# Farama-Foundation/Miniworld

Measured on AMD Instinct MI355X. Metric: env-steps/s (batched, 80x60 RGB), higher is better.
Workload: dtype f32

## Files before the change

include/mwengine.h:

```cpp
#ifndef MWENGINE_H
#define MWENGINE_H
#include <stdint.h>
#ifdef __cplusplus
extern "C" {
#endif

#define MW_ABI_VERSION 4

enum {
    MW_OK = 0,
    MW_E_INVALID = -1,
    MW_E_HIP = -2,
    MW_E_NOMEM = -3,
    MW_E_CAPACITY = -4,
    MW_E_DEVICE = -5,
    MW_E_OVERFLOW = -6
};

enum { MW_ENT_NONE = 0, MW_ENT_BOX = 1, MW_ENT_MESH = 2, MW_ENT_FRAME = 3 };

enum {
    MW_TASK_NONE = 0,
    MW_TASK_GOTO = 1,
    MW_TASK_PICKUP = 2,
// ... 126 lines not shown
typedef struct {
    int32_t n_rooms, n_tex, n_ops, n_ents;
    mw_prog_room rooms[MW_PROG_MAX_ROOMS];
    int32_t tex_nvar[MW_PROG_MAX_TEX];
    int32_t tex_var_id[MW_PROG_MAX_TEX][9];
    double tex_var_scale[MW_PROG_MAX_TEX][9][2];
    mw_prog_op ops[MW_PROG_MAX_OPS];
    int32_t ent_kind[MW_PROG_MAX_ENTS], ent_mesh[MW_PROG_MAX_ENTS], ent_static[MW_PROG_MAX_ENTS];
    double ent_pos[MW_PROG_MAX_ENTS][3], ent_dir[MW_PROG_MAX_ENTS], ent_geom[MW_PROG_MAX_ENTS][9];
    double colors[6][3];
    double extent[4];
    double street[4];
    int32_t sign_n, pad;
    int32_t sign_slot[8];
    double sign_reward[8];
} mw_gen_program;

int mw_set_gen_program(mw_engine *e, const mw_gen_program *prog, const mw_poly *polys, const int32_t *poly_room,
                       const int32_t *poly_surf, const double *poly_m , int32_t n_polys,
                       const double *segs, int32_t n_segs);

int mw_create(const mw_config *cfg, mw_engine **out);
void mw_destroy(mw_engine *e);
const char *mw_last_error(const mw_engine *e);

int mw_upload_texture(mw_engine *e, int32_t tex_id, const uint8_t *rgb_bottom_up, int32_t w, int32_t h);
int mw_upload_mesh(mw_engine *e, int32_t mesh_id, const float *pos, const float *nrm, const float *uv,
                   const float *rgb, int32_t ntris, int32_t tex_id);

int mw_set_geometry(mw_engine *e, int32_t env, const mw_poly *polys, int32_t n_polys,
                    const double *segs, int32_t n_segs);
int mw_get_geometry(mw_engine *e, int32_t env, mw_poly *polys, int32_t *n_polys, double *segs, int32_t *n_segs);
int mw_set_state(mw_engine *e, int32_t first_env, int32_t count, const mw_state_view *host);
int mw_set_step_params(mw_engine *e, const double *host_params);
int mw_get_state(mw_engine *e, int32_t first_env, int32_t count, mw_state_view *host);
int mw_reset(mw_engine *e, const uint8_t *mask, const uint64_t *seeds, void *stream);

int mw_step(mw_engine *e, const int32_t *d_actions, uint8_t *d_obs, float *d_depth,
            float *d_reward, uint8_t *d_term, uint8_t *d_trunc, void *stream);
#define MW_MAX_REPEAT 256
int mw_step_repeat(mw_engine *e, const int32_t *d_actions, int32_t repeat, uint8_t *d_obs, float *d_depth,
                   float *d_reward, uint8_t *d_term, uint8_t *d_trunc, int32_t *d_nsteps, void *stream);
int mw_set_final_obs(mw_engine *e, uint8_t *d_final_obs, float *d_final_depth);
#define MW_MAX_STACK 16
enum { MW_STACK_PAD_RESET = 0, MW_STACK_PAD_ZERO = 1 };
int mw_set_frame_stack(mw_engine *e, int32_t depth, int32_t pad, uint8_t *d_ring, uint8_t *d_final_stack );
int mw_stack_refresh(mw_engine *e, const uint8_t *d_obs, void *stream);
int mw_stack_window(const mw_engine *e, int32_t *first_slot, int64_t *pushes);
enum { MW_OBS_HWC_U8 = 0, MW_OBS_CWH_U8 = 1, MW_OBS_GREY_F64 = 2 };
int mw_set_obs_layout(mw_engine *e, int32_t layout);

int mw_pcg64_draws(uint64_t seed, int32_t n, const int32_t *bounds, double *out);

int mw_selftest_rcp(unsigned long long *bad_per_exp, uint32_t *examples, uint32_t *n);
int mw_selftest_div(unsigned long long *n_bad, uint32_t *examples);
int mw_selftest_sort(const uint32_t *keys, const int32_t *n, int32_t blocks, uint16_t *order);
int mw_selftest_q(unsigned long long *n_bad, uint32_t *examples);
int mw_selftest_sincosf(unsigned long long *sums, unsigned long long n64, unsigned long long *sums64);

int mw_render(mw_engine *e, uint8_t *d_obs, float *d_depth, void *stream);
int mw_render_top(mw_engine *e, uint8_t *d_obs, float *d_depth, int32_t render_agent, void *stream);
int mw_render_view(mw_engine *e, int32_t env, int32_t view_flags, int32_t width, int32_t height, int32_t msaa,
                   uint8_t *d_out, float *d_depth, void *stream);
int mw_visible_ents(mw_engine *e, int32_t first_env, int32_t count, uint8_t *d_vis, void *stream);

int64_t mw_snapshot_bytes(const mw_engine *e, int32_t capacity);
int mw_snapshot_save(mw_engine *e, const int32_t *d_envs, int32_t count, uint8_t *d_snap, int32_t capacity, void *stream);
int mw_snapshot_load(mw_engine *e, const int32_t *d_envs, const int32_t *d_recs, int32_t count,
                     const uint8_t *d_snap, int32_t n_recs, int32_t capacity, void *stream);

int mw_check(mw_engine *e, void *stream);

int mw_kernel_time_ms(mw_engine *e, int32_t reset, double *raster_ms, double *setup_ms, int64_t *launches);

int mw_get_info(mw_engine *e, int32_t *d_health, double *d_ent_pos, int32_t ent_slot, void *stream);
int mw_get_final_info(mw_engine *e, int32_t *d_health, double *d_goal_pos, void *stream);
int mw_get_reset_pending(mw_engine *e, uint8_t *d_out, void *stream);

int mw_set_frame_reuse(mw_engine *e, int32_t on);
int mw_get_frame_clean(mw_engine *e, uint8_t *d_out, void *stream);

int mw_set_frame_cache(mw_engine *e, int32_t slots);
int mw_get_frame_source(mw_engine *e, uint8_t *d_out, void *stream);

int mw_get_list_lengths(mw_engine *e, int32_t first_env, int32_t count, int32_t *host_out, void *stream);

int mw_debug_set_mesh_frame_seq(mw_engine *e, uint32_t seq);
int mw_debug_get_slow_heads(mw_engine *e, uint32_t *host_out, void *stream);

enum { MW_PATH_TILE = 0, MW_PATH_QUAD = 1, MW_PATH_QUAD_MESH = 2, MW_PATH_GENERIC = 3 };
int mw_raster_path(const mw_engine *e);

#ifdef __cplusplus
}
#endif
#endif
```

miniworld_amd/csrc/mw_engine.hip:

```cpp
#include <hip/hip_runtime.h>

#include <algorithm>
#include <cmath>
#include <cstdarg>
#include <cstdio>
#include <cstdlib>
#include <cstring>
#include <memory>
#include <string>
#include <utility>
#include <vector>

#include "mw_assets.h"
#include "mw_device.h"
#include "mw_kernels.h"
#include "mw_rng.h"

#define MW_TIMING_STRIDE 8

extern "C" __global__ void mw_info_kernel(int N, int E, const int32_t *health, const double *epos, int slot, int32_t *out_health, double *out_pos)
{
    const int i = blockIdx.x * blockDim.x + threadIdx.x;
    if (i >= N) return;
    if (out_health) out_health[i] = health[i];
// ... 54 lines not shown
struct Destroy { void operator()(H h) const { (void)destroy(h); } };
template <typename T>
using DevBuf = std::unique_ptr<T, Destroy<void *, hipFree>>;
using Stream = std::unique_ptr<ihipStream_t, Destroy<hipStream_t, hipStreamDestroy>>;
using Event = std::unique_ptr<ihipEvent_t, Destroy<hipEvent_t, hipEventDestroy>>;
}

struct mw_engine {
    mw_config cfg{};
    MwArgs args{};
    MwArgs *d_gen_live = nullptr, *d_gen_spare = nullptr;
    bool spare_mode = false;
    bool side_refill_pending = false;
    MwSpare spare_host{};
    int32_t *d_spare_dummy = nullptr;
    int n_sets = 1;
    std::string err;
    std::vector<DevBuf<void>> fixed;
    std::vector<MwTexDesc> tex_desc;
    std::vector<std::vector<uint32_t>> tex_data;
    DevBuf<uint32_t> d_texels;
    size_t texel_cap = 0;
    MwMeshDesc *d_meshdesc = nullptr;
    std::vector<mwasset::HostMesh> meshes;
    struct MeshPools {
        DevBuf<float> pos, nrm, rgb, uv;
        DevBuf<float> stream, attr;
        DevBuf<float4> vpos;
        DevBuf<uint2> idx;
    } pools;
    int max_mesh_verts = 0, max_mesh_tris = 0;
    bool have_meshes = false, visible_attr_set = false;
    Stream side_stream;
    Event ev_fork;
    struct MeshPath {
        Stream quad_stream;
        Event ev_fork, ev_join;
        DevBuf<uint32_t> view_keys;
        size_t view_keys_bytes = 0;
        DevBuf<uint32_t> keys;
        bool keys_dirty = true;
        DevBuf<int32_t> slow_count;
        int32_t *ent_counter = nullptr;
        DevBuf<uint32_t> slow_envs;
        DevBuf<uint32_t> tile_list;
        DevBuf<uint32_t> ent_list;
        int ent_list_cap = 0;
        uint32_t frame_seq = 1;
        DevBuf<uint32_t> slow_tris; DevBuf<float4> slow_frags; DevBuf<uint32_t> slow_head;
        DevBuf<float> plane_cache;
        int plane_cap = 0;
        static constexpr int mesh_tile_waves = 16384;
        static constexpr int ent_blocks = 512;
        static constexpr int slow_waves = 8192;
    } mp;
    int obs_layout = MW_OBS_HWC_U8;
    float *d_reward_scratch = nullptr;
    uint8_t *d_flag_scratch = nullptr;
    int32_t *d_action_scratch = nullptr;
    uint8_t *d_mask = nullptr;
    double *d_step_override = nullptr;
    bool use_step_override = false;
    bool timing = false;
    int timing_stride = MW_TIMING_STRIDE;
    uint64_t frame_count = 0;
    struct Ev { Event a, b, c; };
    std::vector<Ev> ev_used, ev_free;
    int waves_per_env = 0;
    DevBuf<MwProgram> d_prog;
    DevBuf<mw_poly> d_prog_polys;
    DevBuf<int32_t> d_prog_room, d_prog_surf;
    DevBuf<double> d_prog_m, d_prog_segs;
    int texel_bytes = 4;
    int dbg_flags = 0;
    int last_raster_path = -1;
    bool use_k2q = true;
    bool k2q_ok = false;
    bool generic_raster = false;
    unsigned long long *d_ent_prof = nullptr;
    unsigned long long *d_k2q_prof = nullptr;
    uint8_t *final_obs = nullptr;
    float *final_depth = nullptr;
    int32_t *d_final_list = nullptr;
    bool frame_reuse = false;
    struct { uint8_t *obs = nullptr; float *depth = nullptr; int layout = 0; bool valid = false; } held;
    struct {
        int slots = 0;
        DevBuf<uint8_t> frames;
        DevBuf<float> depth;
        DevBuf<uint64_t> meta;
        DevBuf<MwFcArgs> d_args;
        MwFcArgs args{};
        bool args_stale = true;
        bool with_depth = false;
        bool dirty = true;
    } fc;
    struct {
        int depth = 0, pad = 0, layout = 0, cur = 0;
        uint8_t *ring = nullptr, *final_stack = nullptr;
        size_t frame_bytes = 0;
        int64_t pushes = 0;
        uint8_t *flags = nullptr;
    } stack;
    MwSnapConfig snap_cfg{};
    MwSnapLayout snap_layout{};
    MwSnapTable *d_snap_tab = nullptr;
    int snap_chunks_per_item = 0;
    Event ev_refill_done;
};

namespace {

int fail(mw_engine *e, int code, const char *fmt, ...)
{
    char buf[512];
    va_list ap;
    va_start(ap, fmt);
    vsnprintf(buf, sizeof buf, fmt, ap);
    va_end(ap);
    if (e) e->err = buf; else g_create_error = buf;
    return code;
}

#define HIP_TRY(e, call)                                                                         \
    do {                                                                                         \
        hipError_t _st = (call);                                                                 \
        if (_st != hipSuccess)                                                                   \
            return fail(e, MW_E_HIP, "%s failed: %s (%s:%d)", #call, hipGetErrorString(_st), __FILE__, __LINE__); \
    } while (0)

template <typename T>
int dev_alloc(mw_engine *e, DevBuf<T> &out, size_t count, bool zero = true)
{
    void *p = nullptr;
    const size_t bytes = std::max<size_t>(count, 1) * sizeof(T);
    hipError_t st = hipMalloc(&p, bytes);
    if (st != hipSuccess) return fail(e, MW_E_NOMEM, "hipMalloc(%zu) failed: %s", bytes, hipGetErrorString(st));
    DevBuf<T> buf(static_cast<T *>(p));
    if (zero) {
        st = hipMemset(p, 0, bytes);
        if (st != hipSuccess) return fail(e, MW_E_HIP, "hipMemset failed: %s", hipGetErrorString(st));
    }
    out = std::move(buf);
    return MW_OK;
}

template <typename T>
int fixed_alloc(mw_engine *e, T **out, size_t count)
{
    DevBuf<T> buf;
    if (const int rc = dev_alloc(e, buf, count)) return rc;
    *out = buf.get();
    e->fixed.emplace_back(std::move(buf));
    return MW_OK;
}

template <typename T, typename C>
int grow(mw_engine *e, DevBuf<T> &buf, C &have, C want, size_t unit)
{
    if (want <= have) return MW_OK;
    DevBuf<T> fresh;
    if (const int rc = dev_alloc(e, fresh, (size_t)want * unit / sizeof(T), false)) return rc;
    (void)hipDeviceSynchronize();
    buf = std::move(fresh);
    have = want;
    return MW_OK;
}

hipError_t make_event(Event &out, unsigned flags = hipEventDisableTiming)
{
    hipEvent_t ev = nullptr;
    const hipError_t st = hipEventCreateWithFlags(&ev, flags);
    if (st == hipSuccess) out.reset(ev);
    return st;
}

hipError_t make_stream(Stream &out)
{
    int prio_least = 0, prio_greatest = 0;
    (void)hipDeviceGetStreamPriorityRange(&prio_least, &prio_greatest);
    hipStream_t s = nullptr;
    const hipError_t st = hipStreamCreateWithPriority(&s, hipStreamNonBlocking, prio_least);
    if (st == hipSuccess) out.reset(s);
    return st;
}

auto k1_of(const mw_engine *e, int lanes) -> decltype(&mw_step_setup_kernel)
{
    const bool pcg = e->cfg.rng_mode == MW_RNG_PCG64;
    if (lanes) return pcg ? mw_step_setup_dense_pcg_kernel : mw_step_setup_dense_kernel;
    return pcg ? mw_step_setup_pcg_kernel : mw_step_setup_kernel;
}

auto k1_repeat_of(const mw_engine *e, int lanes) -> decltype(&mw_step_repeat_kernel)
{
    const bool pcg = e->cfg.rng_mode == MW_RNG_PCG64;
    if (lanes) return pcg ? mw_step_repeat_dense_pcg_kernel : mw_step_repeat_dense_kernel;
    return pcg ? mw_step_repeat_pcg_kernel : mw_step_repeat_kernel;
}

template <typename... A>
struct KernelPair {
    void (*plain)(A...);
    void (*sub)(A..., const int32_t *);
};
template <typename... A>
KernelPair<A...> kernel_pair(void (*plain)(A...), void (*sub)(A..., const int32_t *)) { return {plain, sub}; }
#define MW_PAIR(stem) kernel_pair(stem##_kernel, stem##_sub_kernel)

template <typename... A, typename... P>
void launch(const KernelPair<A...> &k, const int32_t *list, dim3 grid, dim3 block, size_t lds, hipStream_t st, P &&...args)
{
    if (list) hipLaunchKernelGGL(k.sub, grid, block, lds, st, std::forward<P>(args)..., list);
    else hipLaunchKernelGGL(k.plain, grid, block, lds, st, std::forward<P>(args)...);
}

auto geom_kernel_of(int L, int msaa)
{
    const bool fixed8 = msaa == 8;
    if (L == 64) return fixed8 ? MW_PAIR(mw_geom_big) : MW_PAIR(mw_geom_big_any);
    return fixed8 ? MW_PAIR(mw_geom) : MW_PAIR(mw_geom_any);
}

auto tile_kernel_of(bool big, bool depth, bool general, bool ragged, bool mesh, bool first)
{
    if (mesh) {
        if (big) return MW_PAIR(mw_raster_big_mesh_wrap);
        if (general) return MW_PAIR(mw_raster_mesh_wrap);
        if (first) return depth ? MW_PAIR(mw_raster_nomesh_depth) : MW_PAIR(mw_raster_nomesh);
        return depth ? MW_PAIR(mw_raster_mesh_depth) : MW_PAIR(mw_raster_mesh);
    }
    if (ragged) return big ? MW_PAIR(mw_raster_big_ragged) : MW_PAIR(mw_raster_ragged);
    if (general) return big ? MW_PAIR(mw_raster_big_wrap) : MW_PAIR(mw_raster_wrap);
    if (big) return depth ? MW_PAIR(mw_raster_big_depth) : MW_PAIR(mw_raster_big);
    return depth ? MW_PAIR(mw_raster_depth) : MW_PAIR(mw_raster);
}

#define MW_DEBUG_BITS 0xFCCF
int raster_flags(const mw_engine *e, int part, uint32_t stamp, bool reuse = false)
{
    return e->dbg_flags | e->obs_layout << 8 | part << 4 | (int)(stamp << 16) | (reuse && stamp == 0u ? MW_RASTER_REUSE : 0);
}
void drop_held_frame(mw_engine *e) { e->held.valid = false; }
void drop_frame_cache(mw_engine *e) { e->fc.dirty = true; }

size_t obs_row_bytes(const mw_engine *e)
{
    return (size_t)e->cfg.obs_width * e->cfg.obs_height * (e->obs_layout == MW_OBS_GREY_F64 ? 8 : 3);
}

int stack_phase(const mw_engine *e) { return (int)((e->stack.pushes + e->stack.depth - 1) % e->stack.depth); }
uint8_t *stack_flags(const mw_engine *e, int half) { return e->stack.flags + (size_t)half * e->cfg.num_envs; }
int stack_check(mw_engine *e, const char *what)
{
    if (e->stack.depth && (e->stack.layout != e->obs_layout || e->stack.frame_bytes != obs_row_bytes(e)))
        return fail(e, MW_E_INVALID, "%s: the frame stack was set under obs layout %d, the engine is in layout %d now (mw_set_frame_stack again, or switch back)",
                    what, e->stack.layout, e->obs_layout);
    return MW_OK;
}
int launch_stack(mw_engine *e, bool push, const uint8_t *d_obs, const uint8_t *term, const uint8_t *trunc, hipStream_t st)
{
    auto &s = e->stack;
    const int N = e->cfg.num_envs, phase = push ? (int)(s.pushes % s.depth) : stack_phase(e);
    const bool installs = e->cfg.generator != MW_GEN_NONE;
    const bool same = installs && e->cfg.autoreset == MW_AUTORESET_SAME_STEP, next = installs && e->cfg.autoreset == MW_AUTORESET_NEXT_STEP;
    const uint8_t *final_obs = push && same && s.final_stack ? e->final_obs : nullptr;
    uint8_t *final_stack = final_obs ? s.final_stack : nullptr;
    const bool wide = (((uintptr_t)d_obs | (uintptr_t)s.ring | (uintptr_t)final_obs | (uintptr_t)final_stack | (uintptr_t)s.frame_bytes) & 15u) == 0;
    const size_t units = s.frame_bytes / (wide ? 16 : 1), chunk = (size_t)MW_STACK_THREADS * MW_STACK_UNROLL;
    const dim3 grid(N, (unsigned)((units + chunk - 1) / chunk));
    const uint8_t *in = stack_flags(e, s.cur);
    uint8_t *out = stack_flags(e, s.cur ^ 1);
    if (push)
        hipLaunchKernelGGL(mw_stack_push_kernel, grid, dim3(MW_STACK_THREADS), 0, st, s.depth, s.pad, phase, (unsigned long long)s.frame_bytes, (int)wide, d_obs, s.ring,
                           in, out, same ? term : nullptr, same ? trunc : nullptr, next ? (const uint8_t *)e->args.reset_pending : nullptr, final_obs, final_stack);
    else
        hipLaunchKernelGGL(mw_stack_refresh_kernel, grid, dim3(MW_STACK_THREADS), 0, st, s.depth, s.pad, phase, (unsigned long long)s.frame_bytes, (int)wide, d_obs, s.ring,
                           in, out);
    HIP_TRY(e, hipGetLastError());
    s.cur ^= 1;
    if (push) ++s.pushes;
    return MW_OK;
}

bool tile_kernels_exact(int W, int H) { return W <= 128 && H <= 128 && W * H <= 128 * 96; }

bool frame_on_grid(int W, int H) { return W % MW_TILE_W == 0 && H % MW_TILE_H == 0; }
bool tile_path_ok(int W, int H) { return frame_on_grid(W, H) && tile_kernels_exact(W, H); }
bool frame_size_ok(int W, int H)
{
    return W >= 1 && H >= 1 && W <= 255 * MW_TILE_W && H <= 255 * MW_TILE_H;
}

int geom_lanes(const mw_engine *e)
{
    const int items = 2 * (e->cfg.max_polys + 6 * e->cfg.max_ents + 1);
    int L = 8;
    while (L < items && L < 64) L <<= 1;
    if (L == 32) L = 16;
    if (L == 64 && !e->args.rec_order && e->cfg.max_polys <= 64) L = 32;
#if defined(MW_PERF_HOOKS) || defined(MW_TUNE_HOOKS)
    if (const char *s = getenv("MW_GEOM_LANES")) { const int v = atoi(s); if ((v == 8 || v == 16 || v == 32 || v == 64) && v >= L) L = v; }
#endif
    return L;
}

// ... 135 lines not shown
}

struct RasterPath {
    int path;
    bool mesh;
    bool quad4;
    bool big, general, ragged, depth;
};
RasterPath raster_path(const mw_engine *e, bool depth)
{
    const MwArgs &a = e->args; const int S = e->cfg.msaa;
    RasterPath p{MW_PATH_GENERIC, false, false, a.rec_order != nullptr, e->obs_layout != MW_OBS_HWC_U8 || e->dbg_flags != 0, !frame_on_grid(a.W, a.H), depth};
    const bool k2q = e->use_k2q && e->k2q_ok && !p.big && !(S == 4 && (e->have_meshes || e->generic_raster));
    const bool ragged_tiles = !e->have_meshes && p.ragged && a.H % 2 == 0 && tile_kernels_exact(a.tiles_x * MW_TILE_W, a.tiles_y * MW_TILE_H);
    p.quad4 = k2q && S == 4;
    const bool generic = S != 8 || (!tile_path_ok(a.W, a.H) && !ragged_tiles);
    p.mesh = !p.quad4 && !generic && e->have_meshes;
    p.path = p.quad4 ? MW_PATH_QUAD : generic ? MW_PATH_GENERIC : !k2q ? MW_PATH_TILE : p.mesh ? MW_PATH_QUAD_MESH : MW_PATH_QUAD;
    return p;
}

int ensure_mesh_buffers(mw_engine *e)
{
    const MwArgs &a = e->args; mw_engine::MeshPath &m = e->mp;
    const size_t N = (size_t)e->cfg.num_envs;
    if (!m.quad_stream) HIP_TRY(e, make_stream(m.quad_stream));
    for (Event *ev : {&m.ev_fork, &m.ev_join}) if (!*ev) HIP_TRY(e, make_event(*ev));
    if (raster_path(e, false).path == MW_PATH_GENERIC)
        return grow(e, m.view_keys, m.view_keys_bytes, N * a.W * a.H * e->cfg.msaa * 4, 1);
    if (a.W > 255 * MW_TILE_W || a.H > 255 * MW_TILE_H) return fail(e, MW_E_CAPACITY, "frame too large for the mesh tile rectangles");
    if (a.n_tiles > 255 || a.n_tiles > 32 * geom_lanes(e))
        return fail(e, MW_E_CAPACITY, "%d tiles per frame: the mesh tiles' work list holds 255 (8-bit tile index) and 32 per lane of the geometry kernel (%d lanes)", a.n_tiles, geom_lanes(e));
    const long long want = std::min<long long>(0xC000, (long long)e->cfg.max_ents * e->max_mesh_tris);
    int rc;
    if ((rc = grow(e, m.plane_cache, m.plane_cap, (int)want, N * (MW_PLANE_REC + MW_PLANE_XTRA) * 4))) return rc;
    if (!m.ent_list) {
        const int cap = (int)N * std::min(MW_MAX_MESH_ENTS, std::max(e->cfg.max_ents, 1));
        DevBuf<uint32_t> ents, slow, tiles;
        if ((rc = dev_alloc(e, ents, (size_t)cap * 16, false)) || (rc = dev_alloc(e, slow, N * 2, false)) ||
            (rc = dev_alloc(e, tiles, N * (size_t)a.n_tiles * 8, false)))
            return rc;
        m.ent_list_cap = cap;
        m.ent_list = std::move(ents); m.slow_envs = std::move(slow); m.tile_list = std::move(tiles);
    }
    if (!m.keys) {
        const size_t px = N * a.W * a.H;
        DevBuf<uint32_t> keys, tris, head; DevBuf<int32_t> cnt; DevBuf<float4> frags;
        if ((rc = dev_alloc(e, keys, px * 8, false)) || (rc = dev_alloc(e, cnt, N * 4 + 2 * MW_CNT_WORDS)) ||
            (rc = dev_alloc(e, tris, N * MW_SLOW_TRIS, false)) || (rc = dev_alloc(e, frags, N * MW_SLOW_STRIDE, false)) ||
            (rc = dev_alloc(e, head, px)))
            return rc;
        HIP_TRY(e, hipMemset(keys.get(), 0xFF, px * 8 * 4));
        m.ent_counter = cnt.get() + N * 4;
        m.keys = std::move(keys); m.slow_count = std::move(cnt); m.slow_tris = std::move(tris);
        m.slow_frags = std::move(frags); m.slow_head = std::move(head);
        (void)hipDeviceSynchronize();
        m.keys_dirty = false;
    }
    return MW_OK;
}

struct MeshFrame {
    uint32_t stamp;
    int parity;
    int32_t *cnt, *cnt_next, *slow_count;
    uint32_t *slow_envs;
};
MeshFrame mesh_frame(mw_engine::MeshPath &m, size_t N)
{
    const uint32_t seq = m.frame_seq++;
    const int parity = (int)(seq & 1u);
    return {seq & 0xFFFFu, parity, m.ent_counter + parity * MW_CNT_WORDS, m.ent_counter + (parity ^ 1) * MW_CNT_WORDS,
            m.slow_count.get() + (size_t)parity * 2 * N, m.slow_envs.get() + (size_t)parity * N};
}

enum { FRAME_ALL = 0, FRAME_TERMINAL = 1, FRAME_LIST = 2 };

struct Frame {
    MwArgs a;
    int view_flags;
    const int32_t *list;
    uint8_t *obs; float *depth; hipStream_t st; bool reuse;
    int fc_slots;
    uint8_t *source;
    RasterPath p;
    MeshFrame mf;
};

void launch_step_and_geometry(mw_engine *e, const Frame &f, bool do_step, int frame, bool async_refill, const int32_t *d_actions,
                              float *d_reward, uint8_t *d_term, uint8_t *d_trunc, int repeat, int32_t *d_nsteps)
{
    const MwArgs &a = f.a; const int N = e->cfg.num_envs;
    if (do_step) {
        const int refill_blocks = (e->spare_mode && !async_refill) ? (N + 63) / 64 : 0;
        MwArgs ak = a;
        if (frame == FRAME_TERMINAL) ak.autoreset = MW_AUTORESET_NEXT_STEP;
        const int lanes = k1_dense_lanes(e), epw = lanes ? 64 / lanes : 1;
        const dim3 grid((N + epw - 1) / epw + refill_blocks);
        float *reward = d_reward ? d_reward : e->d_reward_scratch;
        uint8_t *term = d_term ? d_term : e->d_flag_scratch, *trunc = d_trunc ? d_trunc : e->d_flag_scratch + N;
        if (repeat > 0) hipLaunchKernelGGL(k1_repeat_of(e, lanes), grid, dim3(64), 0, f.st, ak, lanes, d_actions, reward, term, trunc, repeat, d_nsteps);
        else hipLaunchKernelGGL(k1_of(e, lanes), grid, dim3(64), 0, f.st, ak, lanes, d_actions, reward, term, trunc);
    }
    if (frame == FRAME_TERMINAL)
        hipLaunchKernelGGL(mw_final_list_kernel, dim3(1), dim3(1024), 0, f.st, N, (const uint8_t *)a.reset_pending, a.pending_remove, e->d_final_list);
    const int L = geom_lanes(e), epw = 64 / L;
    launch(geom_kernel_of(L, e->cfg.msaa), f.list, dim3((N + epw - 1) / epw), dim3(64), 0, f.st, a, f.view_flags, e->cfg.msaa, L, N);
    if (do_step && e->cfg.task == MW_TASK_COLLECT)
        hipLaunchKernelGGL(e->cfg.rng_mode == MW_RNG_PCG64 ? mw_collect_respawn_pcg_kernel : mw_collect_respawn_kernel, dim3((N + 63) / 64), dim3(64), 0, f.st, a);
}

int launch_side_refill(mw_engine *e, hipStream_t st)
{
    if (!e->side_stream) HIP_TRY(e, make_stream(e->side_stream));
    if (!e->ev_fork) HIP_TRY(e, make_event(e->ev_fork));
    HIP_TRY(e, hipEventRecord(e->ev_fork.get(), st));
    HIP_TRY(e, hipStreamWaitEvent(e->side_stream.get(), e->ev_fork.get(), 0));
    hipLaunchKernelGGL(e->cfg.rng_mode == MW_RNG_PCG64 ? mw_refill_pcg_kernel : mw_refill_kernel, dim3(e->cfg.num_envs), dim3(64), 0, e->side_stream.get(), e->args);
    e->side_refill_pending = true;
    return MW_OK;
}

int launch_generic(mw_engine *e, const MwArgs &a, int first_env, int count, int S, dim3 mesh_grid, uint8_t *out, float *depth,
                   int layout, const int32_t *list, hipStream_t st)
{
    uint32_t *keys = nullptr;
    if (e->have_meshes) {
        const size_t need = (size_t)count * a.W * a.H * S * 4;
        if (need > e->mp.view_keys_bytes) return fail(e, MW_E_INVALID, "view keys missing (mw_upload_mesh allocates them)");
        keys = e->mp.view_keys.get();
        HIP_TRY(e, hipMemsetAsync(keys, 0xFF, need, st));
        launch(MW_PAIR(mw_view_mesh), list, mesh_grid, dim3(256), 0, st, a.W, a.H, S, first_env, (const float *)a.envhdr, a.mesh_pos, keys);
    }
    const bool any = !frame_on_grid(a.W, a.H) || layout != MW_OBS_HWC_U8;
    launch(any ? MW_PAIR(mw_view_raster_any) : MW_PAIR(mw_view_raster), list, dim3(a.n_tiles, count), dim3(64), 0, st, first_env, a.W, a.H, S,
           a.max_vis, a.tiles_x, (const float *)a.rec_raster, (const float *)a.rec_shade, (const float *)a.rec_cull, (const int32_t *)a.nvis,
           (const float *)a.envhdr, a.tex, a.texels, a.mesh_pos, a.mesh_nrm, a.mesh_rgb, a.mesh_uv, keys, out, depth, e->texel_bytes, layout);
    return MW_OK;
}

void launch_quad(const mw_engine *e, const Frame &f, int part, hipStream_t st)
{
    const MwArgs &a = f.a;
    const int lds = mw_rasterq_lds_bytes(e->cfg.msaa, a.W, a.H, a.n_tiles, f.depth ? 1 : 0);
    launch(f.p.quad4 ? MW_PAIR(mw_rasterq4) : MW_PAIR(mw_rasterq), f.list, dim3(e->cfg.num_envs), dim3(MWQ_THREADS), (size_t)lds, st, a.N, a.W, a.H, a.max_vis,
           a.tiles_x, a.n_tiles, (const float *)a.rec_raster, (const float *)a.rec_shade, (const float *)a.rec_cull,
           (const int32_t *)a.nvis, (const float *)a.envhdr, a.texels, f.obs, f.depth, raster_flags(e, part, 0u, f.reuse), e->texel_bytes, e->d_k2q_prof,
           (const uint8_t *)a.frame_clean, f.fc_slots ? (const MwFcArgs *)e->fc.d_args.get() : nullptr, f.source);
}

void launch_tiles(const mw_engine *e, const Frame &f, int part, hipStream_t st)
{
    const MwArgs &a = f.a; const mw_engine::MeshPath &m = e->mp;
    const int N = e->cfg.num_envs, wpe = e->waves_per_env;
    const int lds_recs = a.max_vis < MW_LDS_RECS ? a.max_vis : MW_LDS_RECS;
    const size_t lds = f.p.big ? 192 : (size_t)lds_recs * (MW_LDS_SHADE_Q + MW_LDS_CULL_Q) * 16 + 192;
    const bool listed = part == 2 && a.tile_list != nullptr;
    if (listed) part = 3;
    const int wpe2 = part == 2 ? a.n_tiles : wpe;
    const int tpw2 = part == 2 ? 1 : (a.n_tiles + wpe - 1) / wpe;
    const int grid = listed ? std::min(m.mesh_tile_waves, N * (int)a.n_tiles) : (N + 7) / 8 * 8 * wpe2;
    launch(tile_kernel_of(f.p.big, f.p.depth, f.p.general, f.p.ragged, f.p.mesh, part == 1), f.list, dim3(grid), dim3(64), lds, st,
           a.N, a.W, a.H, a.max_vis, a.tiles_x, a.n_tiles, wpe2, tpw2, (const float *)a.rec_raster, (const float *)a.rec_shade,
           (const float *)a.rec_cull, (const int32_t *)a.nvis, (const float *)a.envhdr, a.tex, a.texels, f.obs, f.depth, raster_flags(e, part, f.mf.stamp, f.reuse),
           e->texel_bytes, (const uint16_t *)a.rec_order, a.mesh_pos, a.mesh_nrm, a.mesh_rgb, a.mesh_uv, m.keys.get(),
           (const float *)m.plane_cache.get(), m.plane_cap, (const float4 *)m.slow_frags.get(), (const uint32_t *)m.slow_head.get(),
           (const uint32_t *)a.tile_list, a.ent_list_n, a.tile_list_cap, std::max(a.n_xcc, 1), (const uint8_t *)a.frame_clean);
}

int launch_mesh_chain(mw_engine *e, const Frame &f, hipStream_t st)
{
    const MwArgs &a = f.a; const MeshFrame &mf = f.mf;
    mw_engine::MeshPath &m = e->mp; const int N = e->cfg.num_envs;
    if (!m.keys || !m.plane_cache || !m.quad_stream) return fail(e, MW_E_INVALID, "mesh buffers missing (mw_upload_mesh allocates them)");
    if (m.keys_dirty) HIP_TRY(e, hipMemsetAsync(m.keys.get(), 0xFF, (size_t)N * a.W * a.H * 8 * 4, st));
    m.keys_dirty = true;
    if (mf.stamp == 0u) HIP_TRY(e, hipMemsetAsync(m.slow_head.get(), 0, (size_t)N * a.W * a.H * 4, st));
    HIP_TRY(e, hipEventRecord(m.ev_fork.get(), st));
    HIP_TRY(e, hipStreamWaitEvent(m.quad_stream.get(), m.ev_fork.get(), 0));
    hipLaunchKernelGGL(mw_mesh_entity_kernel, dim3(std::max(a.n_xcc, std::min(m.ent_list_cap, m.ent_blocks))), dim3(MW_ENT_THREADS), (size_t)e->max_mesh_verts * 16, st, N, a.W, a.H,
                       (const float *)a.envhdr, a.mesh, (const float4 *)e->pools.vpos.get(), (const uint2 *)e->pools.idx.get(), (const float *)e->pools.stream.get(),
                       (const float *)e->pools.attr.get(), m.keys.get(), m.plane_cache.get(), m.plane_cap, mf.slow_count, m.slow_tris.get(),
                       (const uint32_t *)m.ent_list.get(), m.ent_list_cap, mf.cnt, mf.cnt_next, mf.slow_envs, e->args.n_xcc, e->d_ent_prof);
    hipLaunchKernelGGL(mw_mesh_slow_kernel, dim3(std::min(N * 16, m.slow_waves)), dim3(64), 0, st, a.W, a.H, (const float *)a.envhdr, a.mesh_pos, a.mesh_nrm, a.mesh_rgb,
                       a.mesh_uv, a.texels, e->texel_bytes, m.keys.get(), m.slow_count.get(), N, mf.parity, (const uint32_t *)m.slow_tris.get(),
                       m.slow_frags.get(), m.slow_head.get(), mf.stamp, a.status,
                       (const uint32_t *)mf.slow_envs, (const int32_t *)(mf.cnt + MW_CNT_SLOW_ENVS));
    if (f.p.path == MW_PATH_QUAD_MESH) launch_quad(e, f, 1, m.quad_stream.get()); else launch_tiles(e, f, 1, m.quad_stream.get());
    launch_tiles(e, f, 2, st);
    HIP_TRY(e, hipEventRecord(m.ev_join.get(), m.quad_stream.get()));
    HIP_TRY(e, hipStreamWaitEvent(st, m.ev_join.get(), 0));
    m.keys_dirty = false;
    return MW_OK;
}

int launch_frame(mw_engine *e, bool do_step, int view_flags, const int32_t *d_actions, uint8_t *d_obs, float *d_depth,
                 float *d_reward, uint8_t *d_term, uint8_t *d_trunc, hipStream_t st, int frame = FRAME_ALL, int repeat = 0,
                 int32_t *d_nsteps = nullptr)
{
    if (!d_obs) return fail(e, MW_E_INVALID, "d_obs is null");
    const bool plain = frame == FRAME_ALL && view_flags == 0;
    const bool reuse = e->frame_reuse && plain && do_step && !e->have_meshes && e->dbg_flags == 0 && e->held.valid && e->held.obs == d_obs &&
                       e->held.depth == d_depth && e->held.layout == e->obs_layout;
    drop_held_frame(e);
    const int N = e->cfg.num_envs;
    Frame f{e->args, view_flags, frame == FRAME_LIST ? e->d_final_list : nullptr, d_obs, d_depth, st, reuse, 0, nullptr, raster_path(e, d_depth != nullptr), {}};
    if (plain && do_step && f.p.path == MW_PATH_QUAD) {
        f.source = f.a.fc_source;
        if (e->fc.slots > 0 && e->fc.frames && !e->have_meshes && e->dbg_flags == 0 && e->obs_layout == MW_OBS_HWC_U8 && e->cfg.task != MW_TASK_COLLECT) {
            if (d_depth && !e->fc.depth) {
                if (const int rc = dev_alloc(e, e->fc.depth, (size_t)N * e->fc.slots * f.a.W * f.a.H, false)) return rc;
                e->fc.args_stale = true;
            }
            if ((d_depth != nullptr) != e->fc.with_depth) { e->fc.with_depth = d_depth != nullptr; drop_frame_cache(e); }
            if (e->fc.args_stale) {
                e->fc.args = MwFcArgs{f.a.fc_key, e->fc.meta.get(), e->fc.frames.get(), e->fc.depth.get(), e->fc.slots, 0};
                HIP_TRY(e, hipMemcpyAsync(e->fc.d_args.get(), &e->fc.args, sizeof(MwFcArgs), hipMemcpyHostToDevice, st));
                e->fc.args_stale = false;
                drop_frame_cache(e);
            }
            if (e->fc.dirty) {
                HIP_TRY(e, hipMemsetAsync(e->fc.meta.get(), 0, (size_t)N * MW_FC_META_WORDS(e->fc.slots) * 8, st));
                e->fc.dirty = false;
            }
            f.fc_slots = e->fc.slots;
        }
    }
    f.a.step_override = e->use_step_override ? e->d_step_override : nullptr;
    if (f.p.mesh && e->mp.ent_list && e->mp.keys) {
        f.mf = mesh_frame(e->mp, (size_t)N);
        f.a.ent_list = e->mp.ent_list.get(); f.a.ent_list_n = f.mf.cnt; f.a.ent_list_cap = e->mp.ent_list_cap;
        f.a.tile_list = e->mp.tile_list.get(); f.a.tile_list_cap = N * f.a.n_tiles;
    }
    mw_engine::Ev ev{};
    const bool timed = frame != FRAME_LIST && e->timing && (e->frame_count++ % (uint64_t)e->timing_stride) == 0;
    if (timed) {
        ev = get_events(e);
        (void)hipEventRecord(ev.a.get(), st);
    }
    const bool async_refill = e->spare_mode && do_step && e->cfg.generator == MW_GEN_MAZE;
    launch_step_and_geometry(e, f, do_step, frame, async_refill, d_actions, d_reward, d_term, d_trunc, repeat, d_nsteps);
    if (timed) (void)hipEventRecord(ev.b.get(), st);
    int rc = MW_OK;
    if (async_refill && (rc = launch_side_refill(e, st))) return rc;
    if (f.p.path == MW_PATH_GENERIC) rc = launch_generic(e, f.a, 0, N, e->cfg.msaa, dim3(32, N), d_obs, d_depth, e->obs_layout, f.list, st);
    else if (f.p.mesh) rc = launch_mesh_chain(e, f, st);
    else if (f.p.path == MW_PATH_QUAD) launch_quad(e, f, 0, st);
    else launch_tiles(e, f, 0, st);
    if (rc) return rc;
    e->last_raster_path = f.p.path;
    if (timed) {
        (void)hipEventRecord(ev.c.get(), st);
        e->ev_used.push_back(std::move(ev));
    }
    HIP_TRY(e, hipGetLastError());
    if (plain) e->held = {d_obs, d_depth, e->obs_layout, true};
    return MW_OK;
}

int init_engine(mw_engine *e, const mw_config *cfg)
{
    e->cfg = *cfg;
    const int N = cfg->num_envs, E = std::max(cfg->max_ents, 1);
    e->cfg.max_ents = E;
    e->n_sets = cfg->shared_geometry ? 1 : N;
    MwArgs &a = e->args;
    a.N = N; a.W = cfg->obs_width; a.H = cfg->obs_height; a.E = E;
    a.max_polys = cfg->max_polys; a.max_segs = cfg->max_segs;
    a.max_vis = cfg->max_visible * 6 < 60000 ? cfg->max_visible * 6 : 60000;
    a.shared_geom = cfg->shared_geometry ? 1 : 0;
    a.task = cfg->task; a.goal_ent = cfg->goal_ent; a.goal_ent2 = cfg->goal_ent2; a.num_objs = cfg->num_objs; a.max_steps = cfg->max_episode_steps;
    a.rng_mode = cfg->rng_mode;
    a.occlusion = 1;
    if (const char *s = getenv("MW_OCCLUSION")) a.occlusion = atoi(s) != 0;
    a.domain_rand = cfg->domain_rand; a.generator = cfg->generator; a.autoreset = cfg->autoreset;
    a.tiles_x = (a.W + MW_TILE_W - 1) / MW_TILE_W; a.tiles_y = (a.H + MW_TILE_H - 1) / MW_TILE_H; a.n_tiles = a.tiles_x * a.tiles_y;
    a.agent_radius = cfg->agent_radius; a.max_forward_step = cfg->max_forward_step;
    a.agent_height = cfg->agent_height > 0.0 ? cfg->agent_height : 1.6;
    a.fwd = cfg->forward_step; a.drift = cfg->forward_drift; a.turn = cfg->turn_step;
    memcpy(a.gen_args, cfg->gen_args, sizeof a.gen_args);
    MwGenTables gt{};
    memcpy(gt.gen_tab, cfg->gen_tab, sizeof gt.gen_tab);
    memcpy(gt.gen_colors, cfg->gen_colors, sizeof gt.gen_colors);
    memcpy(gt.tex_nvar, cfg->tex_nvar, sizeof gt.tex_nvar);
    memcpy(gt.tex_var_id, cfg->tex_var_id, sizeof gt.tex_var_id);
    memcpy(gt.tex_var_scale, cfg->tex_var_scale, sizeof gt.tex_var_scale);
    gt.room_wall_height = cfg->room_wall_height; gt.room_no_ceiling = cfg->room_no_ceiling;
    for (int i = 0; i < 3; ++i) {
        a.sky[i] = cfg->sky_color[i]; a.light_pos[i] = cfg->light_pos[i]; a.light_color[i] = cfg->light_color[i];
        a.light_ambient[i] = cfg->light_ambient[i]; a.color_bias[i] = cfg->obj_color_bias[i];
    }
    a.cam_height = cfg->cam_height; a.cam_fwd_disp = cfg->cam_fwd_disp; a.cam_pitch = cfg->cam_pitch; a.cam_fov_y = cfg->cam_fov_y;
#define ALLOC(ptr, count) do { if (const int rc_ = fixed_alloc(e, &ptr, (size_t)(count))) return rc_; } while (0)
    ALLOC(a.ax, N); ALLOC(a.ay, N); ALLOC(a.az, N); ALLOC(a.adir, N);
    ALLOC(a.cam, 4 * (size_t)N); ALLOC(a.light, 12 * (size_t)N);
    ALLOC(a.carry, N); ALLOC(a.step, N); ALLOC(a.picked, N);
    if (cfg->task == MW_TASK_COLLECT) { ALLOC(a.health, N); ALLOC(a.final_health, N); }
    ALLOC(a.final_goal, 3 * (size_t)N);
    ALLOC(a.ekind, (size_t)E * N); ALLOC(a.emesh, (size_t)E * N); ALLOC(a.estatic, (size_t)E * N);
    ALLOC(a.epos, 3 * (size_t)E * N); ALLOC(a.edir, (size_t)E * N); ALLOC(a.egeom, 9 * (size_t)E * N);
    ALLOC(a.rng, 5 * (size_t)N); ALLOC(a.extent, 4 * (size_t)N);
    MwGenTables *d_gt = nullptr;
    ALLOC(d_gt, 1);
    HIP_TRY(e, hipMemcpy(d_gt, &gt, sizeof gt, hipMemcpyHostToDevice));
    a.gt = d_gt;
    mw_poly *polys = nullptr; int32_t *npolys = nullptr; double *segs = nullptr; int32_t *nsegs = nullptr;
    ALLOC(polys, (size_t)e->n_sets * cfg->max_polys); ALLOC(npolys, e->n_sets);
    ALLOC(segs, (size_t)e->n_sets * cfg->max_segs * 4); ALLOC(nsegs, e->n_sets);
    a.polys = polys; a.npolys = npolys; a.segs = segs; a.nsegs = nsegs;
    MwSpare sp{};
    {
        const bool small_scene = cfg->max_visible <= 64 && cfg->max_polys + 6 * std::max(cfg->max_ents, 1) <= 32;
        bool want = small_scene || cfg->generator == MW_GEN_MAZE;
        if (const char *s = getenv("MW_SPARE")) want = atoi(s) != 0;
        e->spare_mode = cfg->generator != MW_GEN_NONE && !cfg->domain_rand && want && cfg->task != MW_TASK_COLLECT;
    }
    if (e->spare_mode) {
        ALLOC(sp.ax, N); ALLOC(sp.ay, N); ALLOC(sp.az, N); ALLOC(sp.adir, N);
        ALLOC(sp.cam, 4 * (size_t)N); ALLOC(sp.light, 12 * (size_t)N); ALLOC(sp.extent, 4 * (size_t)N);
        ALLOC(sp.ekind, (size_t)E * N); ALLOC(sp.emesh, (size_t)E * N); ALLOC(sp.estatic, (size_t)E * N);
        ALLOC(sp.epos, 3 * (size_t)E * N); ALLOC(sp.edir, (size_t)E * N); ALLOC(sp.egeom, 9 * (size_t)E * N);
        if (!cfg->shared_geometry) {
            ALLOC(sp.polys, (size_t)e->n_sets * cfg->max_polys); ALLOC(sp.npolys, e->n_sets);
            ALLOC(sp.segs, (size_t)e->n_sets * cfg->max_segs * 4); ALLOC(sp.nsegs, e->n_sets);
        }
        MwSpare *d_sp = nullptr;
        ALLOC(d_sp, 1);
        ALLOC(a.refill_mask, N);
        ALLOC(e->d_spare_dummy, 3 * (size_t)N);
        e->spare_host = sp;
        {
            std::vector<uint32_t> ones((size_t)N, 1u);
            HIP_TRY(e, hipMemcpy(a.refill_mask, ones.data(), 4 * (size_t)N, hipMemcpyHostToDevice));
        }
        HIP_TRY(e, hipMemcpy(d_sp, &sp, sizeof sp, hipMemcpyHostToDevice));
        a.spare = d_sp;
    }
    if (cfg->generator != MW_GEN_NONE) {
        ALLOC(e->d_gen_live, 1); a.gen_live = e->d_gen_live;
        if (e->spare_mode) { ALLOC(e->d_gen_spare, 1); a.gen_spare = e->d_gen_spare; }
    }
    ALLOC(e->d_meshdesc, MW_MAX_MESH);
    a.mesh = e->d_meshdesc;
    ALLOC(a.rec_raster, (size_t)N * a.max_vis * MW_RASTER_REC);
    ALLOC(a.rec_shade, (size_t)N * a.max_vis * MW_SHADE_REC);
    ALLOC(a.rec_cull, (size_t)N * a.max_vis * MW_CULL_REC);
    if (cfg->max_visible > 64) {
        ALLOC(a.rec_order, (size_t)N * (a.max_vis + 1));
    }
    if (cfg->max_polys > 64 && !(getenv("MW_OCC_CACHE") && atoi(getenv("MW_OCC_CACHE")) == 0)) {
        ALLOC(a.occ_valid, e->n_sets);
        ALLOC(a.occ_cache, (size_t)e->n_sets * MW_OCC_CACHE_STRIDE(cfg->max_polys));
    }
    ALLOC(a.pending_remove, (size_t)N);
    ALLOC(a.reset_pending, (size_t)N);
    ALLOC(a.frame_clean, (size_t)N);
    ALLOC(a.fc_key, (size_t)MW_FC_KEY_WORDS * N); ALLOC(a.fc_epoch, (size_t)N); ALLOC(a.fc_source, (size_t)N);
    HIP_TRY(e, hipMemset(a.pending_remove, 0xFF, 4 * (size_t)N));
    ALLOC(a.nvis, N); ALLOC(a.envhdr, (size_t)MW_ENVHDR * N); ALLOC(a.status, 1);
    ALLOC(e->d_reward_scratch, N); ALLOC(e->d_flag_scratch, 2 * (size_t)N); ALLOC(e->d_action_scratch, N);
    ALLOC(e->d_final_list, 1 + (size_t)N);
    ALLOC(e->stack.flags, 2 * (size_t)N);
    ALLOC(e->d_mask, N); ALLOC(e->d_step_override, 3 * (size_t)N);
#ifdef MW_PERF_HOOKS
    if (getenv("MW_K1_PROF")) ALLOC(a.k1_prof, MW_K1_PROF_SLOTS * (size_t)N);
    if (getenv("MW_ENT_PROF")) ALLOC(e->d_ent_prof, (size_t)16 * 2 * N * MW_MAX_MESH_ENTS * 8);
    if (getenv("MW_K2Q_PROF")) ALLOC(e->d_k2q_prof, (size_t)N * 80);
#endif
#undef ALLOC
    {
        std::vector<int32_t> m1((size_t)N, -1);
        HIP_TRY(e, hipMemcpy(a.carry, m1.data(), 4 * (size_t)N, hipMemcpyHostToDevice));
        std::vector<uint64_t> seeds(5 * (size_t)N, 0);
        for (int i = 0; i < N; ++i) seed_env(e, seeds.data(), i, (uint64_t)i);
        HIP_TRY(e, hipMemcpy(a.rng, seeds.data(), 40 * (size_t)N, hipMemcpyHostToDevice));
    }
    e->meshes.assign(MW_MAX_MESH, {}); e->tex_desc.assign(MW_MAX_TEX, MwTexDesc{}); e->tex_data.assign(MW_MAX_TEX, {});
    if (const int rc = upload_textures(e)) return rc;
    e->waves_per_env = pick_waves_per_env(e);
    {
        uint32_t *p = nullptr, ids[256];
        a.n_xcc = 0;
        if (hipMalloc((void **)&p, sizeof ids) == hipSuccess) {
            const DevBuf<uint32_t> d_ids(p);
            hipLaunchKernelGGL(mw_xcc_probe_kernel, dim3(256), dim3(64), 0, 0, d_ids.get());
            if (hipMemcpy(ids, d_ids.get(), sizeof ids, hipMemcpyDeviceToHost) == hipSuccess) {
                uint32_t seen = 0u;
                for (uint32_t v : ids) seen |= 1u << (v & 15u);
                for (int n : {8, 4, 2}) if (seen == (1u << n) - 1u) a.n_xcc = n;
            }
        }
        if (a.n_xcc == 0) a.n_xcc = 1;
    }
    if (const char *s = getenv("MW_DEBUG_FLAGS")) e->dbg_flags = atoi(s) & MW_DEBUG_BITS;
    if (const char *s = getenv("MW_K2Q")) e->use_k2q = atoi(s) != 0;
    if (const char *s = getenv("MW_GENERIC_RASTER")) e->generic_raster = atoi(s) != 0;
    {
        const int S = cfg->msaa == 4 ? 4 : 8;
        const int lds = mw_rasterq_lds_bytes(S, a.W, a.H, a.n_tiles, 1);
        e->k2q_ok = (cfg->msaa == 8 || cfg->msaa == 4) && frame_on_grid(a.W, a.H) && a.W <= 128 && a.H <= 128 && a.W * a.H <= 8192 && lds <= 64 * 1024;
    }
    {
        e->snap_cfg = {E, cfg->max_polys, cfg->max_segs, cfg->shared_geometry ? 1 : 0, cfg->task, cfg->generator, cfg->rng_mode, e->spare_mode ? 1 : 0,
                       cfg->task == MW_TASK_COLLECT ? 1 : 0};
        const MwSnapLayout &L = e->snap_layout = mw_snap_layout(e->snap_cfg);
        void *arr[MW_SC_COUNT] = {};
        arr[MW_SC_AX] = a.ax; arr[MW_SC_AY] = a.ay; arr[MW_SC_AZ] = a.az; arr[MW_SC_ADIR] = a.adir; arr[MW_SC_CAM] = a.cam; arr[MW_SC_LIGHT] = a.light;
        arr[MW_SC_EXTENT] = a.extent; arr[MW_SC_CARRY] = a.carry; arr[MW_SC_STEP] = a.step; arr[MW_SC_PICKED] = a.picked; arr[MW_SC_HEALTH] = a.health;
        arr[MW_SC_FINAL_HEALTH] = a.final_health; arr[MW_SC_FINAL_GOAL] = a.final_goal; arr[MW_SC_EKIND] = a.ekind; arr[MW_SC_EMESH] = a.emesh;
        arr[MW_SC_ESTATIC] = a.estatic; arr[MW_SC_EPOS] = a.epos; arr[MW_SC_EDIR] = a.edir; arr[MW_SC_EGEOM] = a.egeom; arr[MW_SC_RNG] = a.rng;
        arr[MW_SC_PENDING_REMOVE] = a.pending_remove; arr[MW_SC_RESET_PENDING] = a.reset_pending;
        arr[MW_SC_NPOLYS] = const_cast<int32_t *>(a.npolys); arr[MW_SC_NSEGS] = const_cast<int32_t *>(a.nsegs);
        arr[MW_SC_SP_AX] = sp.ax; arr[MW_SC_SP_AY] = sp.ay; arr[MW_SC_SP_AZ] = sp.az; arr[MW_SC_SP_ADIR] = sp.adir; arr[MW_SC_SP_CAM] = sp.cam;
        arr[MW_SC_SP_LIGHT] = sp.light; arr[MW_SC_SP_EXTENT] = sp.extent; arr[MW_SC_SP_EKIND] = sp.ekind; arr[MW_SC_SP_EMESH] = sp.emesh;
        arr[MW_SC_SP_ESTATIC] = sp.estatic; arr[MW_SC_SP_EPOS] = sp.epos; arr[MW_SC_SP_EDIR] = sp.edir; arr[MW_SC_SP_EGEOM] = sp.egeom;
        arr[MW_SC_SP_NPOLYS] = sp.npolys; arr[MW_SC_SP_NSEGS] = sp.nsegs; arr[MW_SC_REFILL_MASK] = a.refill_mask;
        MwSnapTable t{};
        for (int id = 0; id < MW_SC_COUNT; ++id) {
            if (!L.comp_rows[id]) continue;
            if (!arr[id]) return fail(e, MW_E_INVALID, "snapshot layout: component %d has rows but no array", id);
            t.comp[t.n_comps++] = {arr[id], L.comp_unit[id], L.comp_row0[id], L.comp_rows[id], L.comp_elem[id], 0};
        }
        t.total_rows = L.total_rows; t.n_geo = L.n_geo; t.max_polys = cfg->max_polys; t.max_segs = cfg->max_segs;
        const int chunk = MW_SNAP_THREADS * MW_SNAP_UNROLL;
        t.poly_chunks = (cfg->max_polys * (MW_SNAP_POLY_BYTES / 16) + chunk - 1) / chunk;
        t.seg_chunks = (cfg->max_segs * (MW_SNAP_SEG_BYTES / 16) + chunk - 1) / chunk;
        t.eng_polys[0] = const_cast<mw_poly *>(a.polys); t.eng_segs[0] = const_cast<double *>(a.segs);
        t.eng_npolys[0] = const_cast<int32_t *>(a.npolys); t.eng_nsegs[0] = const_cast<int32_t *>(a.nsegs);
        t.eng_polys[1] = sp.polys; t.eng_segs[1] = sp.segs; t.eng_npolys[1] = sp.npolys; t.eng_nsegs[1] = sp.nsegs;
        t.polys_unit[0] = L.blob_unit[MW_SB_POLYS]; t.segs_unit[0] = L.blob_unit[MW_SB_SEGS];
        t.polys_unit[1] = L.blob_unit[MW_SB_SP_POLYS]; t.segs_unit[1] = L.blob_unit[MW_SB_SP_SEGS];
        t.npolys_unit[0] = L.comp_unit[MW_SC_NPOLYS]; t.nsegs_unit[0] = L.comp_unit[MW_SC_NSEGS];
        t.npolys_unit[1] = L.comp_unit[MW_SC_SP_NPOLYS]; t.nsegs_unit[1] = L.comp_unit[MW_SC_SP_NSEGS];
        t.reset_pending_unit = L.comp_unit[MW_SC_RESET_PENDING];
        e->snap_chunks_per_item = t.n_geo * (t.poly_chunks + t.seg_chunks);
        {
            std::vector<uint16_t> row_comp((size_t)t.total_rows);
            for (int c = 0; c < t.n_comps; ++c)
                for (int r = 0; r < t.comp[c].rows; ++r) row_comp[(size_t)t.comp[c].row0 + r] = (uint16_t)c;
            uint16_t *d_row_comp = nullptr;
            if (const int rc = fixed_alloc(e, &d_row_comp, row_comp.size())) return rc;
            HIP_TRY(e, hipMemcpy(d_row_comp, row_comp.data(), row_comp.size() * sizeof(uint16_t), hipMemcpyHostToDevice));
            t.row_comp = d_row_comp;
        }
// ... 601 lines not shown
    ON_DEVICE(e);
    HIP_TRY(e, hipStreamSynchronize((hipStream_t)stream));
    HIP_TRY(e, hipMemcpy(host_out, e->args.nvis + first_env, sizeof(int32_t) * (size_t)count, hipMemcpyDeviceToHost));
    return MW_OK;
}

int mw_get_info(mw_engine *e, int32_t *d_health, double *d_ent_pos, int32_t ent_slot, void *stream)
{
    if (!e) return MW_E_INVALID;
    if (!d_health && !d_ent_pos) return fail(e, MW_E_INVALID, "mw_get_info: nothing asked for");
    if (d_ent_pos && (ent_slot < 0 || ent_slot >= e->args.E)) return fail(e, MW_E_INVALID, "mw_get_info: entity slot %d out of range", ent_slot);
    if (d_health && !e->args.health) return fail(e, MW_E_INVALID, "mw_get_info: this engine's task keeps no health (MW_TASK_COLLECT only)");
    ON_DEVICE(e);
    const int N = e->cfg.num_envs;
    hipLaunchKernelGGL(mw_info_kernel, dim3((N + 255) / 256), dim3(256), 0, (hipStream_t)stream, N, e->args.E, (const int32_t *)e->args.health,
                       (const double *)e->args.epos, d_ent_pos ? ent_slot : 0, d_health, d_ent_pos);
    HIP_TRY(e, hipGetLastError());
    return MW_OK;
}

int mw_get_final_info(mw_engine *e, int32_t *d_health, double *d_goal_pos, void *stream)
{
    if (!e) return MW_E_INVALID;
    if (!d_health && !d_goal_pos) return fail(e, MW_E_INVALID, "mw_get_final_info: nothing asked for");
    if (d_health && !e->args.final_health) return fail(e, MW_E_INVALID, "mw_get_final_info: this engine's task keeps no health (MW_TASK_COLLECT only)");
    ON_DEVICE(e);
    const int N = e->cfg.num_envs;
    hipLaunchKernelGGL(mw_info_kernel, dim3((N + 255) / 256), dim3(256), 0, (hipStream_t)stream, N, 1, (const int32_t *)e->args.final_health,
                       (const double *)e->args.final_goal, 0, d_health, d_goal_pos);
    HIP_TRY(e, hipGetLastError());
    return MW_OK;
}

int mw_get_reset_pending(mw_engine *e, uint8_t *d_out, void *stream)
{
    if (!e) return MW_E_INVALID;
    if (!d_out) return fail(e, MW_E_INVALID, "mw_get_reset_pending: d_out is null");
    ON_DEVICE(e);
    HIP_TRY(e, hipMemcpyAsync(d_out, e->args.reset_pending, (size_t)e->cfg.num_envs, hipMemcpyDeviceToDevice, (hipStream_t)stream));
    return MW_OK;
}

int mw_set_frame_reuse(mw_engine *e, int32_t on)
{
    if (!e) return MW_E_INVALID;
    drop_held_frame(e);
    e->frame_reuse = on != 0;
    return MW_OK;
}

int mw_set_frame_cache(mw_engine *e, int32_t slots)
{
    if (!e) return MW_E_INVALID;
    if (slots < 0 || slots > MW_FC_MAX_SLOTS) return fail(e, MW_E_INVALID, "mw_set_frame_cache: %d slots outside 0 .. %d", (int)slots, MW_FC_MAX_SLOTS);
    ON_DEVICE(e);
    drop_frame_cache(e);
    if (slots == e->fc.slots) return MW_OK;
    HIP_TRY(e, hipDeviceSynchronize());
    e->fc.slots = 0;
    e->fc.frames.reset(); e->fc.depth.reset(); e->fc.meta.reset();
    if (slots > 0 && e->use_k2q && e->k2q_ok) {
        const size_t N = (size_t)e->cfg.num_envs;
        DevBuf<uint8_t> frames; DevBuf<uint64_t> meta;
        int rc;
        if ((rc = dev_alloc(e, frames, N * slots * e->cfg.obs_width * e->cfg.obs_height * 3, false)) || (rc = dev_alloc(e, meta, N * MW_FC_META_WORDS(slots))) ||
            (!e->fc.d_args && (rc = dev_alloc(e, e->fc.d_args, 1))))
            return rc;
        e->fc.frames = std::move(frames); e->fc.meta = std::move(meta);
        e->fc.args_stale = true;
    }
    e->fc.slots = slots;
    return MW_OK;
}

int mw_get_frame_source(mw_engine *e, uint8_t *d_out, void *stream)
{
    if (!e) return MW_E_INVALID;
    if (!d_out) return fail(e, MW_E_INVALID, "mw_get_frame_source: d_out is null");
    ON_DEVICE(e);
    HIP_TRY(e, hipMemcpyAsync(d_out, e->args.fc_source, (size_t)e->cfg.num_envs, hipMemcpyDeviceToDevice, (hipStream_t)stream));
    return MW_OK;
}

int mw_get_frame_clean(mw_engine *e, uint8_t *d_out, void *stream)
{
    if (!e) return MW_E_INVALID;
    if (!d_out) return fail(e, MW_E_INVALID, "mw_get_frame_clean: d_out is null");
    ON_DEVICE(e);
    HIP_TRY(e, hipMemcpyAsync(d_out, e->args.frame_clean, (size_t)e->cfg.num_envs, hipMemcpyDeviceToDevice, (hipStream_t)stream));
    return MW_OK;
}

int mw_kernel_time_ms(mw_engine *e, int32_t reset, double *raster_ms, double *setup_ms, int64_t *launches)
{
    if (!e) return MW_E_INVALID;
    ON_DEVICE(e);
    double r = 0, s = 0;
    int64_t n = 0;
    for (auto &ev : e->ev_used) {
        (void)hipEventSynchronize(ev.c.get());
        float t1 = 0, t2 = 0;
        (void)hipEventElapsedTime(&t1, ev.a.get(), ev.b.get());
        (void)hipEventElapsedTime(&t2, ev.b.get(), ev.c.get());
        s += t1; r += t2; ++n;
        e->ev_free.push_back(std::move(ev));
    }
    e->ev_used.clear();
    if (raster_ms) *raster_ms = n ? r / n : 0.0;
    if (setup_ms) *setup_ms = n ? s / n : 0.0;
    if (launches) *launches = n;
    e->timing = true;
    e->frame_count = 0;
    e->timing_stride = reset > 0 ? reset : MW_TIMING_STRIDE;
    if (reset < 0) e->timing = false;
    return MW_OK;
}

int mw_abi_version(void) { return MW_ABI_VERSION; }

}
```

miniworld_amd/csrc/mw_geom.hip:

```cpp
#include <cstddef>
#include "mw_setup_common.h"
#include "mw_records.h"
#include "mw_kernels.h"

namespace {

constexpr int kClipSlots = 24;

__device__ inline void wave_lds_sync()
{
    __builtin_amdgcn_fence(__ATOMIC_RELEASE, "workgroup", "local");
    __builtin_amdgcn_wave_barrier();
    __builtin_amdgcn_fence(__ATOMIC_ACQUIRE, "workgroup", "local");
}

__device__ inline int group_excl_scan(int v, int sub, int L, int &total)
{
    int x = v;
    for (int off = 1; off < L; off <<= 1) {
        const int y = __shfl_up(x, off, L);
        if (sub >= off) x += y;
    }
    total = __shfl(x, L - 1, L);
    return x - v;
// ... 43 lines not shown
                for (int r = 0; r < R; ++r) {
                    if (r & jj) continue;
                    const bool up = ((64 * r) & k) == 0;
                    const uint32_t lo = min(x[r], x[r ^ jj]), hi = max(x[r], x[r ^ jj]);
                    x[r] = up ? lo : hi; x[r ^ jj] = up ? hi : lo;
                }
            } else {
#pragma unroll
                for (int r = 0; r < R; ++r) {
                    const uint32_t y = (uint32_t)__shfl_xor((int)x[r], j);
                    const bool up = (((64 * r) | lane) & k) == 0;
                    const bool keep_min = ((lane & j) == 0) == up;
                    x[r] = keep_min ? min(x[r], y) : max(x[r], y);
                }
            }
        }
    }
#pragma unroll
    for (int r = 0; r < R; ++r)
        if (64 * r + lane < n) order[1 + 64 * r + lane] = (uint16_t)(x[r] & 0xFFFFu);
}

#define MW_OCC_BINS 256
#define MW_OCC_CAP 192
#define MW_ORDER_CAP 512

__device__ inline bool occluded_span(const float *occ_z, float xlo, float xhi, float zq, float bins_per_px)
{
    const float fb0 = floorf(fmaxf(xlo, 0.0f) * bins_per_px), fb1 = floorf(fmaxf(xhi, 0.0f) * bins_per_px);
    const int b0 = (int)fminf(fb0, (float)(MW_OCC_BINS - 1)), b1 = (int)fminf(fb1, (float)(MW_OCC_BINS - 1));
    const float thr = zq * __builtin_amdgcn_rcpf(fmaf(1.2e-3f, zq, 1.0f)) * 0.9999f;
    const int g0 = (b0 + 15) >> 4, g1 = (b1 + 1) >> 4;
    if (g0 >= g1) {
        for (int b = b0; b <= b1; ++b)
            if (!(occ_z[b] < thr)) return false;
        return true;
    }
    for (int b = b0; b < (g0 << 4); ++b)
        if (!(occ_z[b] < thr)) return false;
    for (int g = g0; g < g1; ++g)
        if (!(occ_z[MW_OCC_BINS + g] < thr)) return false;
    for (int b = g1 << 4; b <= b1; ++b)
        if (!(occ_z[b] < thr)) return false;
    return true;
}

__device__ inline bool occluded(const float *occ_z, const mwgl::Vert v[4], float bins_per_px)
{
    float zq = 1e30f, xmn = 1e30f, xmx = -1e30f;
    bool ok = true;
#pragma unroll
    for (int k = 0; k < 4; ++k) {
        ok &= v[k].clip[3] >= 0.1f;
        xmn = fminf(xmn, v[k].win[0]); xmx = fmaxf(xmx, v[k].win[0]); zq = fminf(zq, v[k].clip[3]);
    }
    return ok && occluded_span(occ_z, xmn - 0.1f, xmx + 0.1f, zq, bins_per_px);
}

__device__ inline bool occluded_span_rmq(const float *rmq, float xlo, float xhi, float zq, float bins_per_px)
{
    const float fb0 = floorf(fmaxf(xlo, 0.0f) * bins_per_px), fb1 = floorf(fmaxf(xhi, 0.0f) * bins_per_px);
    const int b0 = (int)fminf(fb0, (float)(MW_OCC_BINS - 1)), b1 = (int)fminf(fb1, (float)(MW_OCC_BINS - 1));
    const float thr = zq * __builtin_amdgcn_rcpf(fmaf(1.2e-3f, zq, 1.0f)) * 0.9999f;
    if (b1 < b0) return true;
    const int k = 31 - __builtin_clz((unsigned)(b1 - b0 + 1));
    const float m = fmaxf(rmq[k * MW_OCC_BINS + b0], rmq[k * MW_OCC_BINS + b1 - (1 << k) + 1]);
    return m < thr;
}

__device__ inline bool occluded_rmq(const float *rmq, const mwgl::Vert v[4], float bins_per_px)
{
    float zq = 1e30f, xmn = 1e30f, xmx = -1e30f;
    bool ok = true;
#pragma unroll
    for (int k = 0; k < 4; ++k) {
        ok &= v[k].clip[3] >= 0.1f;
        xmn = fminf(xmn, v[k].win[0]); xmx = fmaxf(xmx, v[k].win[0]); zq = fminf(zq, v[k].clip[3]);
    }
    return ok && occluded_span_rmq(rmq, xmn - 0.1f, xmx + 0.1f, zq, bins_per_px);
}

}

template <bool BIG, int SFIX, bool SUB = false>
__device__ inline void geom_body(const MwArgs &a, int view_flags, int S_, int L, int n_env, const int32_t *__restrict__ list = nullptr)
{
    const int S = SFIX ? SFIX : S_;
    struct ClipSlot { mwgl::ClipVert l[2][MWGL_MAX_CLIP_VERTS]; float pad[4]; };
    __shared__ ClipSlot s_clip[kClipSlots];
    __shared__ int s_pos[BIG ? 1 : 8][66];
    __shared__ uint32_t s_meta[64], s_res[64];
    __shared__ float s_occ_z[BIG ? MW_OCC_BINS + MW_OCC_BINS / 16 : 1];
    __shared__ int s_occ_n;
    float *s_rmq = reinterpret_cast<float *>(&s_clip[0]);
    float4 *s_occ_wall = reinterpret_cast<float4 *>(s_rmq + 9 * MW_OCC_BINS);
    static_assert(!BIG || sizeof(ClipSlot) * kClipSlots >= (9 * MW_OCC_BINS + 8 * MW_OCC_CAP) * sizeof(float), "the sift borrows the clipper's LDS");
    __shared__ uint16_t s_list[BIG ? 4096 : 1];
    __shared__ uint32_t s_key[BIG ? MW_ORDER_CAP : 1];
#ifdef MW_PERF_HOOKS
#define KGP_ON (a.k1_prof != nullptr)
#else
#define KGP_ON false
#endif
    const unsigned long long tstart = KGP_ON ? __builtin_readcyclecounter() : 0ull;
    const unsigned long long rt_start = KGP_ON ? __builtin_amdgcn_s_memrealtime() : 0ull;
    [[maybe_unused]] unsigned long long ts[4] = {0, 0, 0, 0};
    [[maybe_unused]] int kp_nocc = 0, kp_nkept = 0, kp_nclip = 0;
    [[maybe_unused]] unsigned long long kp_clip = 0, kp_emit = 0, kp_e_shfl = 0, kp_e_setup = 0, kp_e_write = 0;
    const int lane = threadIdx.x;
    const int epw = 64 / L, sub = lane & (L - 1), grp = lane / L;
    if (SUB) {
        n_env = list[0];
        if ((int)blockIdx.x * epw >= n_env) return;
    }
    const int rel = (int)blockIdx.x * epw + grp;
    const bool live = rel < n_env;
    const int env = SUB ? list[1 + (live ? rel : n_env - 1)] : a.env_base + (live ? rel : n_env - 1);
    const int set = a.shared_geom ? 0 : env;
    const bool top = (view_flags & 1) != 0, proxy = (view_flags & 4) != 0, ms = S > 1;
    constexpr int kWallPf = BIG ? 4 : 1;
    float4 pf_wall[kWallPf], pf_box0 = make_float4(0.0f, 0.0f, 0.0f, 0.0f), pf_box1 = pf_box0;
    float pf_sgn[kWallPf], pf_hdr[3] = {0.0f, 0.0f, 0.0f};
    auto prefetch_occ = [&]() {
        if (!BIG || L != 64 || a.occ_cache == nullptr) return;
        const float *pc = a.occ_cache + (size_t)set * MW_OCC_CACHE_STRIDE(a.max_polys);
#pragma unroll
        for (int q = 0; q < kWallPf; ++q) {
            const int i = lane + 64 * q;
            if (i < a.max_polys) {
                pf_wall[q] = reinterpret_cast<const float4 *>(pc + MW_OCC_CACHE_HDR + 8 * (size_t)i)[0];
                pf_sgn[q] = pc[MW_OCC_CACHE_HDR + 8 * (size_t)i + 4];
            }
        }
        if (lane < (a.max_polys + 7) / 8) {
            const float4 *b4 = reinterpret_cast<const float4 *>(pc + MW_OCC_CACHE_HDR + 8 * (size_t)a.max_polys + 8 * (size_t)lane);
            pf_box0 = b4[0]; pf_box1 = b4[1];
        }
        pf_hdr[0] = pc[0]; pf_hdr[1] = pc[1]; pf_hdr[2] = pc[2];
    };
#pragma unroll
    for (int q = 0; q < kWallPf; ++q) { pf_wall[q] = make_float4(0.0f, 0.0f, 0.0f, 0.0f); pf_sgn[q] = 0.0f; }
    prefetch_occ();
    const bool ent_pre = a.E <= L;
    const int my_ekind = (ent_pre && sub < a.E) ? a.ekind[(size_t)sub * a.N + env] : 0;
    const int my_estatic = (ent_pre && sub < a.E) ? a.estatic[(size_t)sub * a.N + env] : 0;
    const int my_emesh = (ent_pre && sub < a.E && my_ekind == MW_ENT_MESH) ? a.emesh[(size_t)sub * a.N + env] : 0;
    const int my_mesh_ntris = (ent_pre && sub < a.E && my_ekind == MW_ENT_MESH) ? (int)a.mesh[my_emesh].ntris : 0;
    auto ent_kind = [&](int s0) { return ent_pre ? __shfl(my_ekind, s0, L) : a.ekind[(size_t)s0 * a.N + env]; };
    auto ent_static = [&](int s0) { return ent_pre ? __shfl(my_estatic, s0, L) : a.estatic[(size_t)s0 * a.N + env]; };
    auto ent_mesh_ntris = [&](int s0) { return ent_pre ? __shfl(my_mesh_ntris, s0, L) : (int)a.mesh[a.emesh[(size_t)s0 * a.N + env]].ntris; };
    mwgl::Frame f;
    const double px = a.ax[env], py = a.ay[env], pz = a.az[env], dir = a.adir[env];
    float eye_x = 0.0f, eye_y = 0.0f, eye_z = 0.0f;
    {
        double lpos[3], lcol[3], lamb[3];
#pragma unroll
        for (int i = 0; i < 3; ++i) {
            lpos[i] = a.light[(size_t)(3 + i) * a.N + env];
            lcol[i] = a.light[(size_t)(6 + i) * a.N + env];
            lamb[i] = a.light[(size_t)(9 + i) * a.N + env];
        }
        if (top) {
            double min_x = a.extent[(size_t)0 * a.N + env] - 1, max_x = a.extent[(size_t)1 * a.N + env] + 1;
            double min_z = a.extent[(size_t)2 * a.N + env] - 1, max_z = a.extent[(size_t)3 * a.N + env] + 1;
            const double width = max_x - min_x, height = max_z - min_z;
            const double aspect = width / height, fb_aspect = (double)a.W / (double)a.H;
            if (aspect > fb_aspect) {
                const double new_h = width / fb_aspect, h_diff = new_h - height;
                min_z -= h_diff / 2; max_z += h_diff / 2;
            } else if (aspect < fb_aspect) {
                const double new_w = height * fb_aspect, w_diff = new_w - width;
                min_x -= w_diff / 2; max_x += w_diff / 2;
            }
            mwgl::frame_top(f, min_x, max_x, min_z, max_z);
        } else {
            const double cam_height = a.cam[(size_t)0 * a.N + env], fwd_disp = a.cam[(size_t)1 * a.N + env];
            const double pitch_deg = a.cam[(size_t)2 * a.N + env], fov_y = a.cam[(size_t)3 * a.N + env];
            const mw::SinCos hd = mw::sincos_det(dir / 2.0);
            const double ya = hd.c, yc = -1.0 * hd.s;
            const double ry00 = ya * ya - yc * yc, ry02 = 2.0 * (ya * yc), ry11 = ya * ya + yc * yc;
            const double pitch = pitch_deg * kPi / 180.0;
            const mw::SinCos hp = mw::sincos_det(pitch / 2.0);
            const double za = hp.c, zd = -1.0 * hp.s;
            const double rz00 = za * za - zd * zd, rz01 = 2.0 * (0.0 - za * zd);
            const double eye[3] = {px + fwd_disp * ry00, py + cam_height * ry11, pz + fwd_disp * ry02};
            const double cd[3] = {rz00 * ry00, rz01 * ry11, rz00 * ry02};
            const double at[3] = {eye[0] + cd[0], eye[1] + cd[1], eye[2] + cd[2]};
            const mw::SinCos hf = mw::sincos_det(fov_y / 2 * kPi / 180);
            mwgl::frame_perspective(f, eye, at, hf.c / hf.s, a.W, a.H);
            eye_x = (float)eye[0]; eye_y = (float)eye[1]; eye_z = (float)eye[2];
        }
        mwgl::frame_finish(f, a.W, a.H, lpos, lcol, lamb);
    }
    mwgl::Xform cam;
    mwgl::make_xform(f, f.view, f.view_flags, cam);
    unsigned long long tp[8] = {0, 0, 0, 0, 0, 0, 0, 0};
    [[maybe_unused]] unsigned long long racc[8] = {0, 0, 0, 0, 0, 0, 0, 0}, tprev = 0, rstart = 0, rtot[2] = {0, 0}, rvert[2] = {0, 0};
#define KGP_R(k) do { if (KGP_ON) { const unsigned long long n_ = __builtin_readcyclecounter(); racc[k] += n_ - tprev; tprev = n_; } } while (0)
    if (KGP_ON) tp[0] = __builtin_readcyclecounter();

// ... 771 lines not shown
        uint16_t *order = a.rec_order + (size_t)env * (a.max_vis + 1);
        const int n = count;
        if (n > MW_ORDER_CAP || n > a.max_vis || !live) {
            if (lane == 0 && live) order[0] = 0;
        } else {
            wave_lds_sync();
            if (n <= 64) sort_store_keys<1>(s_key, n, lane, order);
            else if (n <= 128) sort_store_keys<2>(s_key, n, lane, order);
            else if (n <= 256) sort_store_keys<4>(s_key, n, lane, order);
            else sort_store_keys<8>(s_key, n, lane, order);
            if (lane == 0) order[0] = 1;
        }
    }
    if (KGP_ON && sub == 0 && live) {
        unsigned long long *pp = a.k1_prof + (size_t)env * MW_K1_PROF_SLOTS;
        pp[0] = tp[0] - tstart; pp[1] = tp[1] - tp[0]; for (int i = 2; i < 7; ++i) pp[i] = racc[i];
        pp[7] = __builtin_readcyclecounter() - tprev;
        pp[20] = rtot[0]; pp[21] = rtot[1]; pp[22] = rvert[0]; pp[23] = rvert[1];
        pp[24] = kp_clip; pp[25] = kp_emit; pp[26] = (unsigned long long)kp_nclip; pp[27] = 0; pp[28] = kp_e_shfl; pp[29] = kp_e_setup; pp[30] = kp_e_write;
        pp[8] = rt_start; pp[9] = __builtin_amdgcn_s_memrealtime();
        pp[10] = (unsigned long long)np; pp[11] = (unsigned long long)npd; pp[12] = (unsigned long long)count; pp[13] = (unsigned long long)n_rounds;
        pp[14] = (unsigned long long)kp_nocc; pp[15] = (unsigned long long)kp_nkept;
        pp[16] = ts[0] - tp[0]; pp[17] = ts[1] - ts[0]; pp[18] = ts[2] - ts[1]; pp[19] = ts[3] - ts[2];
    }
    if (ent_pre && my_mesh_j >= 0 && live) {
        const int nb = total_boxes < 64 ? total_boxes : 64;
        const int end_pos = marker ? pos[nb] : count;
        const int p0 = my_boxes_before < nb ? pos[my_boxes_before] : end_pos;
        hdr[MW_HDR_MESH + MW_HDR_MESH_STRIDE * my_mesh_j + 1] = __int_as_float(p0 + my_tris_before);
    }
    if (sub == 0 && live) {
        a.nvis[env] = count < a.max_vis ? count : a.max_vis;
        hdr[0] = (float)a.light[(size_t)0 * a.N + env]; hdr[1] = (float)a.light[(size_t)1 * a.N + env]; hdr[2] = (float)a.light[(size_t)2 * a.N + env];
        hdr[3] = __int_as_float(total_meshes);
#pragma unroll
        for (int i = 0; i < 3; ++i) { hdr[4 + i] = f.l_amb[i]; hdr[8 + i] = f.l_dif[i]; }
        const int nb = total_boxes < 64 ? total_boxes : 64;
        const int end_pos = marker ? pos[nb] : count;
        if (!ent_pre) {
            for (int j = 0; j < total_meshes; ++j) {
                float *m = hdr + MW_HDR_MESH + MW_HDR_MESH_STRIDE * j;
                const int before = __float_as_int(m[1]);
                const int p0 = before < nb ? pos[before] : end_pos;
                m[1] = __int_as_float(p0 + __float_as_int(m[25]));
            }
        }
        if (count + total_mesh_tris >= 0xFFF0) atomicOr(a.status, MW_ST_VIS_OVERFLOW);
        if (a.ent_list && total_meshes > 0) {
            const int nbig = __popc(big_mask);
            const int xl = env % a.n_xcc;
            int ib = nbig ? atomicAdd(a.ent_list_n + MW_CNT_LONG + xl, nbig) : 0;
            int is = total_meshes - nbig ? atomicAdd(a.ent_list_n + MW_CNT_SHORT + xl, total_meshes - nbig) : 0;
            uint32_t *l_long = a.ent_list + (size_t)xl * a.ent_list_cap, *l_short = a.ent_list + (size_t)(8 + xl) * a.ent_list_cap;
            for (int j = 0; j < total_meshes; ++j) {
                const uint32_t item = (uint32_t)env | ((uint32_t)j << 24);
                if ((big_mask >> j) & 1u) { if (ib < a.ent_list_cap) l_long[ib] = item; ++ib; }
                else { if (is < a.ent_list_cap) l_short[is] = item; ++is; }
            }
        }
        const int rs = a.pending_remove[env];
        if (rs >= 0 && !proxy && a.task != MW_TASK_COLLECT) {
            a.ekind[(size_t)rs * a.N + env] = MW_ENT_NONE;
            a.pending_remove[env] = MW_REMOVE_APPLIED;
        }
    }
    if (a.tile_list) {
        int total;
        const int cnt = live ? __popc(tile_mask) : 0, excl = group_excl_scan(cnt, sub, L, total);
        int o = 0;
        const int xl = env % a.n_xcc;
        if (sub == 0 && total > 0) o = atomicAdd(a.ent_list_n + MW_CNT_TILES + xl, total);
        o = __shfl(o, 0, L) + excl;
        uint32_t *list = a.tile_list + (size_t)xl * a.tile_list_cap;
        for (uint32_t m = live ? tile_mask : 0u; m; m &= m - 1u, ++o)
            if (o < a.tile_list_cap) list[o] = (uint32_t)env | ((uint32_t)(sub + (__ffs((int)m) - 1) * L) << 24);
    }
}

#ifndef MW_GEOM_OCC
#define MW_GEOM_OCC
#endif
#define MW_GEOM_PAIR(stem, bounds, ...)                                                                                        \
    extern "C" __global__ bounds void stem##_kernel(MW_GEOM_ARGS) { geom_body<__VA_ARGS__, false>(a, view_flags, S, L, n_env); } \
    extern "C" __global__ bounds void stem##_sub_kernel(MW_GEOM_ARGS, const int32_t *list) { geom_body<__VA_ARGS__, true>(a, view_flags, S, L, n_env, list); }
MW_GEOM_PAIR(mw_geom, __launch_bounds__(64) MW_GEOM_OCC, false, 8)
MW_GEOM_PAIR(mw_geom_big, __launch_bounds__(64) MW_GEOM_OCC, true, 8)
MW_GEOM_PAIR(mw_geom_any, __launch_bounds__(64), false, 0)
MW_GEOM_PAIR(mw_geom_big_any, __launch_bounds__(64), true, 0)

extern "C" __global__ __launch_bounds__(64) void mw_selftest_sort_kernel(const uint32_t *keys, const int32_t *n, uint16_t *order)
{
    __shared__ uint32_t s_key[MW_ORDER_CAP];
    const int lane = threadIdx.x, cnt = n[blockIdx.x];
    for (int i = lane; i < cnt; i += 64) s_key[i] = keys[(size_t)blockIdx.x * MW_ORDER_CAP + i];
    __syncthreads();
    uint16_t *out = order + (size_t)blockIdx.x * (MW_ORDER_CAP + 1);
    if (cnt <= 64) sort_store_keys<1>(s_key, cnt, lane, out);
    else if (cnt <= 128) sort_store_keys<2>(s_key, cnt, lane, out);
    else if (cnt <= 256) sort_store_keys<4>(s_key, cnt, lane, out);
    else sort_store_keys<8>(s_key, cnt, lane, out);
}

extern "C" int mw_selftest_sort(const uint32_t *host_keys , const int32_t *host_n , int32_t blocks, uint16_t *host_order )
{
    uint32_t *d_keys = nullptr; int32_t *d_n = nullptr; uint16_t *d_order = nullptr;
    const size_t kb = (size_t)blocks * MW_ORDER_CAP * 4, ob = (size_t)blocks * (MW_ORDER_CAP + 1) * 2;
    if (blocks <= 0 || hipMalloc((void **)&d_keys, kb) != hipSuccess || hipMalloc((void **)&d_n, (size_t)blocks * 4) != hipSuccess ||
        hipMalloc((void **)&d_order, ob) != hipSuccess) return -1;
    (void)hipMemcpy(d_keys, host_keys, kb, hipMemcpyHostToDevice);
    (void)hipMemcpy(d_n, host_n, (size_t)blocks * 4, hipMemcpyHostToDevice);
    (void)hipMemset(d_order, 0, ob);
    hipLaunchKernelGGL(mw_selftest_sort_kernel, dim3(blocks), dim3(64), 0, 0, d_keys, d_n, d_order);
    const int rc = hipDeviceSynchronize() == hipSuccess ? 0 : -2;
    (void)hipMemcpy(host_order, d_order, ob, hipMemcpyDeviceToHost);
    (void)hipFree(d_keys); (void)hipFree(d_n); (void)hipFree(d_order);
    return rc;
}
```

miniworld_amd/csrc/mw_kernels.h:

```cpp
#pragma once
#include "mw_device.h"
#include "mw_snapshot.h"

#define MW_KERNEL_PAIR(stem, ...)                          \
    extern "C" __global__ void stem##_kernel(__VA_ARGS__); \
    extern "C" __global__ void stem##_sub_kernel(__VA_ARGS__, const int32_t *list)

#define MW_K1_ARGS MwArgs a, int lanes_per_env, const int32_t *__restrict__ actions, float *__restrict__ reward, \
                   uint8_t *__restrict__ term, uint8_t *__restrict__ trunc
extern "C" __global__ void mw_step_setup_kernel(MW_K1_ARGS);
extern "C" __global__ void mw_step_setup_pcg_kernel(MW_K1_ARGS);
extern "C" __global__ void mw_step_setup_dense_kernel(MW_K1_ARGS);
extern "C" __global__ void mw_step_setup_dense_pcg_kernel(MW_K1_ARGS);
#define MW_K1_REPEAT_ARGS MW_K1_ARGS, int repeat, int32_t *__restrict__ nsteps
extern "C" __global__ void mw_step_repeat_kernel(MW_K1_REPEAT_ARGS);
extern "C" __global__ void mw_step_repeat_pcg_kernel(MW_K1_REPEAT_ARGS);
extern "C" __global__ void mw_step_repeat_dense_kernel(MW_K1_REPEAT_ARGS);
extern "C" __global__ void mw_step_repeat_dense_pcg_kernel(MW_K1_REPEAT_ARGS);

extern "C" __global__ void mw_reset_kernel(MwArgs a, const uint8_t *__restrict__ mask, int force_all, int mark_refill);
extern "C" __global__ void mw_reset_pcg_kernel(MwArgs a, const uint8_t *__restrict__ mask, int force_all, int mark_refill);
extern "C" __global__ void mw_refill_kernel(MwArgs a);
extern "C" __global__ void mw_refill_pcg_kernel(MwArgs a);
extern "C" __global__ void mw_collect_respawn_kernel(MwArgs a);
extern "C" __global__ void mw_collect_respawn_pcg_kernel(MwArgs a);
extern "C" __global__ void mw_final_install_kernel(MwArgs a, const int32_t *__restrict__ list);
extern "C" __global__ void mw_final_install_pcg_kernel(MwArgs a, const int32_t *__restrict__ list);
extern "C" __global__ void mw_take_spare_kernel(MwArgs a, const uint8_t *__restrict__ mask, int force_all);

#define MW_GEOM_ARGS MwArgs a, int view_flags, int S, int L, int n_env
MW_KERNEL_PAIR(mw_geom, MW_GEOM_ARGS);
MW_KERNEL_PAIR(mw_geom_big, MW_GEOM_ARGS);
MW_KERNEL_PAIR(mw_geom_any, MW_GEOM_ARGS);
MW_KERNEL_PAIR(mw_geom_big_any, MW_GEOM_ARGS);

#define MW_RASTER_REUSE 0x10000

#define MW_RASTER_ARGS \
    int N, int W, int H, int max_vis, int tiles_x, int n_tiles, int waves_per_env, int tiles_per_wave, \
    const float *__restrict__ rec_raster, const float *__restrict__ rec_shade, const float *__restrict__ rec_cull, \
    const int32_t *__restrict__ nvis_arr, const float *__restrict__ envhdr, const MwTexDesc *__restrict__ texd, \
    const uint32_t *__restrict__ texels, uint8_t *__restrict__ obs, float *__restrict__ depth, int dbg, int texel_bytes, \
    const uint16_t *__restrict__ rec_order, const float *__restrict__ mesh_pos, const float *__restrict__ mesh_nrm, \
    const float *__restrict__ mesh_rgb, const float *__restrict__ mesh_uv, uint32_t *__restrict__ mesh_keys, \
    const float *__restrict__ plane_cache, int plane_cap, const float4 *__restrict__ slow_frags, const uint32_t *__restrict__ slow_head, \
    const uint32_t *__restrict__ tile_list, int32_t *__restrict__ tile_n, int tile_list_cap, int n_xcc, \
    const uint8_t *__restrict__ frame_clean
MW_KERNEL_PAIR(mw_raster, MW_RASTER_ARGS);
MW_KERNEL_PAIR(mw_raster_depth, MW_RASTER_ARGS);
MW_KERNEL_PAIR(mw_raster_big, MW_RASTER_ARGS);
MW_KERNEL_PAIR(mw_raster_big_depth, MW_RASTER_ARGS);
MW_KERNEL_PAIR(mw_raster_wrap, MW_RASTER_ARGS);
MW_KERNEL_PAIR(mw_raster_big_wrap, MW_RASTER_ARGS);
MW_KERNEL_PAIR(mw_raster_ragged, MW_RASTER_ARGS);
MW_KERNEL_PAIR(mw_raster_big_ragged, MW_RASTER_ARGS);
MW_KERNEL_PAIR(mw_raster_nomesh, MW_RASTER_ARGS);
MW_KERNEL_PAIR(mw_raster_nomesh_depth, MW_RASTER_ARGS);
MW_KERNEL_PAIR(mw_raster_mesh, MW_RASTER_ARGS);
MW_KERNEL_PAIR(mw_raster_mesh_depth, MW_RASTER_ARGS);
MW_KERNEL_PAIR(mw_raster_mesh_wrap, MW_RASTER_ARGS);
MW_KERNEL_PAIR(mw_raster_big_mesh_wrap, MW_RASTER_ARGS);

#define MWQ_THREADS 512
#define MWQ_ARGS \
    int N, int W, int H, int max_vis, int tiles_x, int n_tiles, \
    const float *__restrict__ rec_raster, const float *__restrict__ rec_shade, const float *__restrict__ rec_cull, \
    const int32_t *__restrict__ nvis_arr, const float *__restrict__ envhdr, const uint32_t *__restrict__ texels, \
    uint8_t *__restrict__ obs, float *__restrict__ depth, int dbg, int texel_bytes, unsigned long long *__restrict__ prof, \
    const uint8_t *__restrict__ frame_clean, const MwFcArgs *__restrict__ fc, uint8_t *__restrict__ frame_source
MW_KERNEL_PAIR(mw_rasterq, MWQ_ARGS);
MW_KERNEL_PAIR(mw_rasterq4, MWQ_ARGS);
extern "C" int mw_rasterq_lds_bytes(int S, int W, int H, int n_tiles, int depth);
extern "C" int mw_rasterq_cap(int depth);

extern "C" __global__ void mw_mesh_entity_kernel(
    int N, int W, int H, const float *__restrict__ envhdr, const MwMeshDesc *__restrict__ meshes, const float4 *__restrict__ mesh_vpos,
    const uint2 *__restrict__ mesh_idx, const float *__restrict__ mesh_stream, const float *__restrict__ mesh_attr, uint32_t *__restrict__ keys_all,
    float *__restrict__ plane_cache, int plane_cap, int32_t *__restrict__ slow_count, uint32_t *__restrict__ slow_tris, const uint32_t *__restrict__ ent_list,
    int ent_list_cap, int32_t *ent_n, int32_t *ent_n_after, uint32_t *__restrict__ slow_envs, int n_xcc, unsigned long long *prof);
extern "C" __global__ void mw_mesh_slow_kernel(int W, int H, const float *envhdr, const float *mesh_pos, const float *mesh_nrm, const float *mesh_rgb,
                                               const float *mesh_uv, const uint32_t *texels, int texel_bytes, uint32_t *keys, int32_t *counts, int N,
                                               int parity, const uint32_t *slow_tris, float4 *frags, uint32_t *heads, uint32_t stamp, uint32_t *status,
                                               const uint32_t *slow_envs, const int32_t *slow_env_n);
extern "C" __global__ void mw_xcc_probe_kernel(uint32_t *out);

MW_KERNEL_PAIR(mw_view_mesh, int W, int H, int S, int first_env, const float *__restrict__ envhdr, const float *__restrict__ mesh_pos, uint32_t *keys);
#define MW_VIEW_RASTER_ARGS \
    int first_env, int W, int H, int S, int max_vis, int tiles_x, const float *__restrict__ rec_raster, \
    const float *__restrict__ rec_shade, const float *__restrict__ rec_cull, const int32_t *__restrict__ nvis_arr, const float *__restrict__ envhdr, \
    const MwTexDesc *__restrict__ texd, const uint32_t *__restrict__ texels, const float *__restrict__ mesh_pos, \
    const float *__restrict__ mesh_nrm, const float *__restrict__ mesh_rgb, const float *__restrict__ mesh_uv, const uint32_t *mesh_keys, \
    uint8_t *__restrict__ out, float *__restrict__ depth, int texel_bytes, int layout
MW_KERNEL_PAIR(mw_view_raster, MW_VIEW_RASTER_ARGS);
MW_KERNEL_PAIR(mw_view_raster_any, MW_VIEW_RASTER_ARGS);

#define MW_STACK_THREADS 256
#define MW_STACK_UNROLL 4
#define MW_STACK_FRESH 1
#define MW_STACK_PENDING 2
#define MW_STACK_ARGS \
    int depth, int pad, int phase, unsigned long long frame_bytes, int wide, const uint8_t *__restrict__ obs, uint8_t *ring, \
    const uint8_t *__restrict__ flags_in, uint8_t *__restrict__ flags_out
extern "C" __global__ void mw_stack_push_kernel(MW_STACK_ARGS, const uint8_t *__restrict__ term, const uint8_t *__restrict__ trunc,
                                                const uint8_t *__restrict__ pending, const uint8_t *__restrict__ final_obs,
                                                uint8_t *__restrict__ final_stack);
extern "C" __global__ void mw_stack_refresh_kernel(MW_STACK_ARGS);
extern "C" __global__ void mw_stack_mark_kernel(int N, const uint8_t *__restrict__ mask, int force_all, uint8_t *__restrict__ flags);

#define MW_SNAP_ARGS \
    const MwSnapTable *__restrict__ tab, MwSnapKey key, int N, int capacity, int count, int item_chunks, const int32_t *__restrict__ d_envs, \
    uint32_t *__restrict__ status
extern "C" __global__ void mw_snapshot_save_kernel(MW_SNAP_ARGS, uint8_t *__restrict__ snap);
extern "C" __global__ void mw_snapshot_load_kernel(MW_SNAP_ARGS, const uint8_t *__restrict__ snap, const int32_t *__restrict__ d_recs, int n_recs,
                                                   uint8_t *__restrict__ frame_clean, int32_t *__restrict__ occ_valid, uint8_t *__restrict__ stack_flags);

extern "C" __global__ void mw_visible_kernel(int env_base, int W, int H, int S, int max_vis, int E, const float *__restrict__ rec_raster,
                                             const float *__restrict__ rec_cull, const int32_t *__restrict__ nvis, uint8_t *__restrict__ vis);
```

miniworld_amd/csrc/mw_rasterq.hip:

```cpp
#include "mw_mesh.h"
#include "mw_kernels.h"

#define MWQ_WAVES (MWQ_THREADS / 64)
#define MWQ_CAP_MAX 48
#define MWQ_SLOTS 16
#define MWQ_EMPTY 63u
#ifndef MWQ_TILE_FALLBACK
#define MWQ_TILE_FALLBACK 1
#endif
#ifndef MWQ_OCC
#define MWQ_OCC 6
#endif

namespace {

__device__ inline bool wave_all(bool p) { return __builtin_amdgcn_ballot_w64(p) == __builtin_amdgcn_read_exec(); }
__device__ inline bool wave_any(bool p) { return __builtin_amdgcn_ballot_w64(p) != 0ull; }

enum { QC_FALLBACK = 0, QC_BIG, QC_EXACT, QC_P4, QC_P3, QC_P2, QC_P1, QC_TRIV, QC_SKY, QC_NCLS, QC_NONE = 15 };

template <int S> struct QRec {
    static constexpr int TQ = (S + 3) / 4;
    static constexpr int SH = 4 + 3 * TQ;
    static constexpr int CT = SH + 6;
// ... 375 lines not shown
        for (int s = 0; s < S; ++s) any_m |= in_m[s];
        if (!any_m) continue;
        uint32_t bits = 0u;
#pragma unroll
        for (int s = S - 1; s >= 0; --s)
            asm("v_addc_co_u32_e64 %0, vcc, %0, %0, %1" : "+v"(bits) : "s"(in_m[s]) : "vcc");
        cont |= (bits & covbits) != 0u;
        covbits |= bits;
        const RGB c = shade_lane(rec + QRec<S>::SH, cx.te, fx + 0.5f, fy + 0.5f);
#pragma unroll
        for (int s = 0; s < S; ++s) {
            q.r[s] = sel_mask(in_m[s], c.r, q.r[s]);
            q.g[s] = sel_mask(in_m[s], c.g, q.g[s]);
            q.b[s] = sel_mask(in_m[s], c.b, q.b[s]);
        }
        if (cx.depth) {
            const float4 a2 = rec[2], a3 = rec[3];
            z16 = sel_mask(in_m[0], depth16_s<S>(a2.z, a2.w, a3.x, fx, fy, 0), z16);
        }
    }
    const bool qc = wave_any(cont) ? quad_any(cont) : false;
    store_pixel<S>(cx, q, z16, px, py, on && !qc);
    return qc;
}

template <int S, class Tri, class RecOf>
__device__ inline void batch_exact(const QCtx &cx, int kmax, Tri tri, RecOf recp, int px, int py, bool on)
{
    const int gy = cx.H - 1 - py;
    const float fx = (float)px, fy = (float)gy;
    uint32_t key[S];
#pragma unroll
    for (int s = 0; s < S; ++s) key[s] = 0xFFFFFFFFu;
    for (int k = 0; k < kmax; ++k) {
        int p = 0;
        const bool valid = tri(k, p);
        const uint64_t vm = __ballot(valid);
        if (!vm) continue;
        const float4 *rec = recp(valid ? p : 0);
        uint64_t in_m[S];
        cover_lane<S>(rec, px, gy, vm, in_m);
        uint64_t any_m = 0ull;
#pragma unroll
        for (int s = 0; s < S; ++s) any_m |= in_m[s];
        if (!any_m) continue;
        const float4 a2 = rec[2], a3 = rec[3];
#pragma unroll
        for (int s = 0; s < S; ++s) {
            const uint32_t kk = (depth16_s<S>(a2.z, a2.w, a3.x, fx, fy, s) << 16) | (uint32_t)p;
            key[s] = sel_mask(in_m[s], min(key[s], kk), key[s]);
        }
    }
    SmpQ<S> q;
#pragma unroll
    for (int s = 0; s < S; ++s) { q.r[s] = cx.sky_r; q.g[s] = cx.sky_g; q.b[s] = cx.sky_b; }
    uint32_t pid[S];
#pragma unroll
    for (int s = 0; s < S; ++s) pid[s] = key[s] == 0xFFFFFFFFu ? 0x10000u : (key[s] & 0xFFFFu);
    for (int k = 0; k < kmax; ++k) {
        int p = 0;
        const bool valid = tri(k, p);
        bool wins = false;
#pragma unroll
        for (int s = 0; s < S; ++s) wins |= pid[s] == (uint32_t)p;
        wins &= valid;
        if (!wave_any(wins)) continue;
        const float4 *rec = recp(valid ? p : 0);
        const RGB c = shade_lane(rec + QRec<S>::SH, cx.te, fx + 0.5f, fy + 0.5f);
#pragma unroll
        for (int s = 0; s < S; ++s) {
            const bool eq = valid && pid[s] == (uint32_t)p;
            q.r[s] = eq ? c.r : q.r[s]; q.g[s] = eq ? c.g : q.g[s]; q.b[s] = eq ? c.b : q.b[s];
        }
    }
    store_pixel<S>(cx, q, key[0] >> 16, px, py, on);
}

template <int S, bool SUB = false>
__device__ inline void rasterq_body(
    int N, int W, int H, int max_vis, int tiles_x, int n_tiles,
    const float *__restrict__ rec_raster, const float *__restrict__ rec_shade, const float *__restrict__ rec_cull,
    const int32_t *__restrict__ nvis_arr, const float *__restrict__ envhdr, const uint32_t *__restrict__ texels,
    uint8_t *__restrict__ obs, float *__restrict__ depth, int dbg, int texel_bytes, unsigned long long *__restrict__ prof,
    const uint8_t *__restrict__ frame_clean, const MwFcArgs *__restrict__ fc, uint8_t *__restrict__ frame_source,
    const int32_t *__restrict__ list = nullptr)
{
    extern __shared__ __attribute__((aligned(16))) unsigned char smem[];
    typedef QRec<S> R;
    int env = blockIdx.x;
    if (SUB) {
        if (env >= list[0]) return;
        env = list[1 + env];
    } else if (env >= N) return;
    if (!SUB && (dbg & MW_RASTER_REUSE) && frame_clean[env]) {
        if (frame_source && threadIdx.x == 0) frame_source[env] = 1;
        return;
    }
    const int tid = threadIdx.x, lane = tid & 63, wave = tid >> 6;
    const bool has_depth = depth != nullptr;
    uint32_t fc_victim = 0u;
    if (!SUB && fc) {
        const int fc_slots = fc->slots;
        const uint64_t *meta = fc->meta + (size_t)env * MW_FC_META_WORDS(fc_slots);
        const uint4 *cur = reinterpret_cast<const uint4 *>(fc->key + (size_t)env * MW_FC_KEY_WORDS);
        bool eq = false;
        uint4 k = make_uint4(0u, 0u, 0u, 0u);
        if (lane < fc_slots * (MW_FC_KEY_WORDS / 2)) {
            const uint4 c = cur[lane % (MW_FC_KEY_WORDS / 2)];
            k = reinterpret_cast<const uint4 *>(meta + 2)[lane];
            eq = k.x == c.x && k.y == c.y && k.z == c.z && k.w == c.w;
        } else if (lane == 63) k = reinterpret_cast<const uint4 *>(meta)[0];
        const uint64_t m = __builtin_amdgcn_ballot_w64(eq);
        int hit = -1;
        for (int j = fc_slots - 1; j >= 0; --j)
            if (((m >> (j * (MW_FC_KEY_WORDS / 2))) & 31ull) == 31ull) hit = j;
        if (hit >= 0) {
            const int fbytes = W * H * 3;
            const uint8_t *src = fc->frames + ((size_t)env * fc_slots + hit) * fbytes;
            uint8_t *dst = obs + (size_t)env * fbytes;
            if ((reinterpret_cast<uintptr_t>(dst) & 15u) == 0u)
                for (int i = tid; i < fbytes / 16; i += MWQ_THREADS) reinterpret_cast<uint4 *>(dst)[i] = reinterpret_cast<const uint4 *>(src)[i];
            else if ((reinterpret_cast<uintptr_t>(dst) & 3u) == 0u)
                for (int i = tid; i < fbytes / 4; i += MWQ_THREADS) reinterpret_cast<uint32_t *>(dst)[i] = reinterpret_cast<const uint32_t *>(src)[i];
            else
                for (int i = tid; i < fbytes; i += MWQ_THREADS) dst[i] = src[i];
            if (has_depth) {
                const float *zs = fc->depth + ((size_t)env * fc_slots + hit) * (W * H);
                float *zd = depth + (size_t)env * (W * H);
                if ((reinterpret_cast<uintptr_t>(zd) & 15u) == 0u)
                    for (int i = tid; i < W * H / 4; i += MWQ_THREADS) reinterpret_cast<float4 *>(zd)[i] = reinterpret_cast<const float4 *>(zs)[i];
                else
                    for (int i = tid; i < W * H; i += MWQ_THREADS) zd[i] = zs[i];
            }
            if (frame_source && tid == 0) frame_source[env] = (uint8_t)(2 + hit);
            return;
        }
        fc_victim = min((uint32_t)__builtin_amdgcn_readlane((int)k.x, 63), (uint32_t)(fc_slots - 1));
    }
    const QPlan pl = q_plan(S, W, H, n_tiles, has_depth);
    float4 *s_rec = reinterpret_cast<float4 *>(smem + pl.rec);
    uint8_t *s_frame = smem + pl.frame;
    uint16_t *s_z = reinterpret_cast<uint16_t *>(smem + pl.zbuf);
    uint32_t *s_qids = reinterpret_cast<uint32_t *>(smem + pl.qids);
    uint16_t *s_queue = reinterpret_cast<uint16_t *>(smem + pl.queue);
    uint16_t *s_xq = reinterpret_cast<uint16_t *>(smem + pl.xq);
    uint32_t *s_tcnt = reinterpret_cast<uint32_t *>(smem + pl.tcnt);
    uint32_t *s_tfull = reinterpret_cast<uint32_t *>(smem + pl.tfull);
    uint8_t *s_tlist = smem + pl.tlist;
    uint32_t *s_tmask = reinterpret_cast<uint32_t *>(smem + pl.tmask);
    uint32_t *s_pe = reinterpret_cast<uint32_t *>(smem + pl.pe);
    uint32_t *s_misc = reinterpret_cast<uint32_t *>(smem + pl.misc);
    uint16_t *s_rank = reinterpret_cast<uint16_t *>(s_frame);
    uint32_t *s_btab = reinterpret_cast<uint32_t *>(smem + pl.btab);
    const int QW = W / 2, QH = H / 2, nquads = QW * QH;
    const uint32_t m_qw = 0xFFFFFFFFu / (uint32_t)QW + 1u , m_tx = mw_magic16((uint32_t)tiles_x);
    const float *hdr = envhdr + (size_t)env * MW_ENVHDR;
    const int nvis = nvis_arr[env];
    const int part_mode = (dbg >> 4) & 3;
    const bool mesh_env = part_mode == 1 && __float_as_int(hdr[3]) != 0;
    const float *g_rr = rec_raster + (size_t)env * max_vis * MW_RASTER_REC;
    const float4 *g_shade = reinterpret_cast<const float4 *>(rec_shade + (size_t)env * max_vis * MW_SHADE_REC);
    const float4 *g_cull = reinterpret_cast<const float4 *>(rec_cull + (size_t)env * max_vis * MW_CULL_REC);
    const MwTexDesc *texd = reinterpret_cast<const MwTexDesc *>(texels);

    auto stamp = [&](int k) { if (prof && lane == 0) prof[((size_t)env * MWQ_WAVES + wave) * 8 + k] = __builtin_amdgcn_s_memtime(); };
    stamp(0);
    QCtx cx;
    cx.s_rec = s_rec; cx.s_frame = s_frame; cx.s_z = s_z;
    cx.te.tx = __builtin_amdgcn_make_buffer_rsrc((void *)texels, 0, texel_bytes, MW_RSRC_WORD3);
    cx.te.td = cx.te.tx; cx.te.texd = texd; cx.te.flat = dbg & 1;
    cx.sky_r = hdr[0]; cx.sky_g = hdr[1]; cx.sky_b = hdr[2];
    cx.W = W; cx.H = H; cx.depth = has_depth;

    auto stage_quad = [&](int p, int q, float4 *dst, bool with_tex) {
        float4 v;
        if (q < 4) v = reinterpret_cast<const float4 *>(g_rr + (size_t)p * MW_RASTER_REC)[q];
        else if (q < R::SH) { const int k = (q - 4) / R::TQ, j = (q - 4) % R::TQ; v = reinterpret_cast<const float4 *>(g_rr + (size_t)p * MW_RASTER_REC)[4 + 4 * k + j]; }
        else if (q < R::CT) {
            const int j = q - R::SH;
            v = g_shade[(size_t)p * (MW_SHADE_REC / 4) + j];
            if (with_tex && j >= 1 && j <= 4) {
                const int tex = __float_as_int(g_shade[(size_t)p * (MW_SHADE_REC / 4)].w);
                uint32_t w0 = 1u, h0 = 1u, nl = 1u;
                if (tex >= 0) { w0 = texd[tex].w; h0 = texd[tex].h; nl = texd[tex].nlevels; }
                if (j == 1) {
                    const uint32_t pot = ((w0 & (w0 - 1u)) | (h0 & (h0 - 1u))) == 0u ? 1u : 0u;
                    v.w = __uint_as_float((uint32_t)(31 - __builtin_clz(w0)) | ((uint32_t)(31 - __builtin_clz(h0)) << 5) | (nl << 10) | (pot << 15));
                } else if (j == 4) v.w = __uint_as_float(tex >= 0 ? ((uint32_t)tex * (uint32_t)(sizeof(MwTexDesc) / 4) + 4u) * 4u : 0u);
                else v.w = j == 2 ? (float)w0 : (float)h0;
            }
        } else {
            const float4 *rr = reinterpret_cast<const float4 *>(g_rr + (size_t)p * MW_RASTER_REC);
            const float4 r0 = rr[0], r1 = rr[1], r3 = rr[3], tm = g_cull[(size_t)p * (MW_CULL_REC / 4) + 3];
            const int A[3] = {__float_as_int(r0.x), __float_as_int(r0.y), __float_as_int(r0.z)}, B[3] = {__float_as_int(r0.w), __float_as_int(r1.x), __float_as_int(r1.y)};
            const int tmx[3] = {__float_as_int(r3.y), __float_as_int(r3.z), __float_as_int(r3.w)}, tmn[3] = {__float_as_int(tm.x), __float_as_int(tm.y), __float_as_int(tm.z)};
            int c[12];
#pragma unroll
            for (int k = 0; k < 3; ++k) {
                const int ap = max(A[k], 0), an = min(A[k], 0), bp = max(B[k], 0), bn = min(B[k], 0);
                c[k] = tmn[k] - ap * (MW_TILE_W - 1) - bp * (MW_TILE_H - 1);
                c[3 + k] = tmx[k] - an * (MW_TILE_W - 1) - bn * (MW_TILE_H - 1);
                c[6 + k] = tmn[k] - ap - bp;
                c[9 + k] = tmx[k] - an - bn;
            }
            const int j = q - R::CT;
            v = make_float4(__int_as_float(j == 0 ? c[0] : (j == 1 ? c[4] : c[8])), __int_as_float(j == 0 ? c[1] : (j == 1 ? c[5] : c[9])),
                            __int_as_float(j == 0 ? c[2] : (j == 1 ? c[6] : c[10])), __int_as_float(j == 0 ? c[3] : (j == 1 ? c[7] : c[11])));
        }
        *dst = v;
    };

    if (nvis > ((dbg & 0x80) ? 8 : q_cap(has_depth))) {
        if constexpr (S == 8 && MWQ_TILE_FALLBACK) {
            TileCtx tc;
            tc.s_shade = g_shade; tc.s_cull = g_cull; tc.shade_stride = MW_SHADE_REC / 4; tc.cull_stride = MW_CULL_REC / 4;
            tc.rr_env = g_rr; tc.s_pack = smem + wave * 192; tc.hdr = hdr; tc.ment = hdr + MW_HDR_MESH;
            tc.mesh_pos = tc.mesh_nrm = tc.mesh_rgb = tc.mesh_uv = nullptr; tc.planes = nullptr; tc.planes_xtra = nullptr; tc.clipbuf = nullptr; tc.slow_frags = nullptr; tc.slow_head = nullptr;
            tc.slow_stamp = 0u; tc.obs = obs; tc.depth = depth;
            tc.obs_rsrc = __builtin_amdgcn_make_buffer_rsrc((void *)(obs + (size_t)env * H * W * 3), 0, H * W * 3, MW_RSRC_WORD3);
            tc.te = cx.te; tc.sky_r = cx.sky_r; tc.sky_g = cx.sky_g; tc.sky_b = cx.sky_b;
            tc.env = env; tc.nvis = nvis; tc.W = W; tc.H = H; tc.dbg = dbg & ~0xF0; tc.lane = lane;
// ... 236 lines not shown
            if (lane == 0) b = atomicAdd(&s_misc[19], 1u);
            b = (uint32_t)__builtin_amdgcn_readfirstlane((int)b);
            if (b * 16u >= nx) break;
            const bool on = b * 16u + (uint32_t)(lane >> 2) < nx;
            const int Q = on ? (int)s_xq[b * 16u + (uint32_t)(lane >> 2)] : 0;
            const int qy = (int)__umulhi((uint32_t)Q, m_qw), qx = Q - qy * QW;
            const int px = qx * 2 + (lane & 1), py = qy * 2 + ((lane >> 1) & 1);
            const uint32_t ids = on ? s_qids[Q] : 0u;
            auto tri = [&](int k, int &p) { p = (int)((ids >> (6 * k)) & 63u); return p != (int)MWQ_EMPTY; };
            auto recp = [&](int p) { return (const float4 *)(s_rec + p * R::NQ); };
            batch_exact<S>(cx, 4, tri, recp, px, py, on);
        }
        __syncthreads();
    }

    const int fmt = (dbg >> 8) & 3;
    const int npix = W * H;
    auto in_mesh_tile = [&](int px, int py) { return mesh_env && tile_in_mesh_rect(hdr, px / MW_TILE_W, py / MW_TILE_H); };
    if (fmt == 0) {
        uint8_t *dst = obs + (size_t)env * npix * 3;
        if (!mesh_env && (reinterpret_cast<uintptr_t>(dst) & 15u) == 0u) {
            const uint4 *src = reinterpret_cast<const uint4 *>(s_frame);
            for (int i = tid; i < npix * 3 / 16; i += MWQ_THREADS) reinterpret_cast<uint4 *>(dst)[i] = src[i];
        } else if ((reinterpret_cast<uintptr_t>(dst) & 3u) == 0u) {
            const uint32_t *src = reinterpret_cast<const uint32_t *>(s_frame);
            for (int i = tid; i < npix * 3 / 4; i += MWQ_THREADS) {
                const int pix = (i * 4) / 3;
                if (!in_mesh_tile(pix % W, pix / W)) reinterpret_cast<uint32_t *>(dst)[i] = src[i];
            }
        } else {
            for (int i = tid; i < npix * 3; i += MWQ_THREADS) {
                const int pix = i / 3;
                if (!in_mesh_tile(pix % W, pix / W)) dst[i] = s_frame[i];
            }
        }
    } else if (fmt == 1) {
        uint8_t *dst = obs + (size_t)env * npix * 3;
        for (int i = tid; i < npix * 3; i += MWQ_THREADS) {
            const int ch = i / npix, r = i - ch * npix, x = r / H, y = r - x * H;
            if (!in_mesh_tile(x, y)) dst[i] = s_frame[(y * W + x) * 3 + ch];
        }
    } else {
        double *dst = reinterpret_cast<double *>(obs) + (size_t)env * npix;
        for (int i = tid; i < npix; i += MWQ_THREADS) {
            if (in_mesh_tile(i % W, i / W)) continue;
            const double Rv = (double)s_frame[i * 3], Gv = (double)s_frame[i * 3 + 1], Bv = (double)s_frame[i * 3 + 2];
            dst[i] = (0.30 * Rv + 0.59 * Gv) + 0.11 * Bv;
        }
    }
    stamp(7);
    auto depth_of = [&](int i) {
        const float z = (float)s_z[i];
        const float d = z / 65535.0f;
        const float clip = (d - 0.5f) * 2.0f;
        const float den = clip * (float)(100.0 - 0.04) - (float)(100.0 + 0.04);
        return (float)(-2.0 * 100.0 * 0.04) / den;
    };
    if (has_depth) {
        float *dst = depth + (size_t)env * npix;
        for (int i = tid; i < npix; i += MWQ_THREADS) {
            if (in_mesh_tile(i % W, i / W)) continue;
            dst[i] = depth_of(i);
        }
    }
    if (!SUB && fc) {
        const int fc_slots = fc->slots;
        const uint32_t victim = s_misc[20];
        uint64_t *meta = fc->meta + (size_t)env * MW_FC_META_WORDS(fc_slots);
        uint4 *fd = reinterpret_cast<uint4 *>(fc->frames + ((size_t)env * fc_slots + victim) * (npix * 3));
        const uint4 *src = reinterpret_cast<const uint4 *>(s_frame);
        for (int i = tid; i < npix * 3 / 16; i += MWQ_THREADS) fd[i] = src[i];
        if (has_depth) {
            float *fz = fc->depth + ((size_t)env * fc_slots + victim) * npix;
            for (int i = tid; i < npix; i += MWQ_THREADS) fz[i] = depth_of(i);
        }
        if (tid < MW_FC_KEY_WORDS / 2)
            reinterpret_cast<uint4 *>(meta + 2 + MW_FC_KEY_WORDS * victim)[tid] = reinterpret_cast<const uint4 *>(fc->key + (size_t)env * MW_FC_KEY_WORDS)[tid];
        if (tid == 64) meta[0] = (uint64_t)(victim + 1u == (uint32_t)fc_slots ? 0u : victim + 1u);
    }
}

}

#define MWQ_FWD N, W, H, max_vis, tiles_x, n_tiles, rec_raster, rec_shade, rec_cull, nvis_arr, envhdr, texels, obs, depth, dbg, texel_bytes, prof, frame_clean, fc, frame_source
#define MWQ_PAIR(stem, bounds, ...)                                                                          \
    extern "C" __global__ bounds void stem##_kernel(MWQ_ARGS) { rasterq_body<__VA_ARGS__, false>(MWQ_FWD); } \
    extern "C" __global__ bounds void stem##_sub_kernel(MWQ_ARGS, const int32_t *__restrict__ list) { rasterq_body<__VA_ARGS__, true>(MWQ_FWD, list); }
MWQ_PAIR(mw_rasterq, __launch_bounds__(MWQ_THREADS, MWQ_OCC), 8)
MWQ_PAIR(mw_rasterq4, __launch_bounds__(MWQ_THREADS), 4)

extern "C" int mw_rasterq_lds_bytes(int S, int W, int H, int n_tiles, int depth) { return q_plan(S, W, H, n_tiles, depth != 0).total; }
extern "C" int mw_rasterq_cap(int depth) { return q_cap(depth != 0); }

#ifdef MWQ_PROBE
extern "C" __global__ __launch_bounds__(MWQ_THREADS) void mwq_probe_trivial(const uint32_t *texels, int texel_bytes, int W, int H, const uint32_t *ids_in, float sky, int dbg)
{
    extern __shared__ __attribute__((aligned(16))) unsigned char smem[];
    QCtx cx;
    cx.s_rec = reinterpret_cast<float4 *>(smem); cx.s_frame = smem + 20000; cx.s_z = reinterpret_cast<uint16_t *>(smem + 40000);
    cx.te.tx = __builtin_amdgcn_make_buffer_rsrc((void *)texels, 0, texel_bytes, MW_RSRC_WORD3);
    cx.te.td = cx.te.tx; cx.te.texd = nullptr; cx.te.flat = dbg & 1;
    cx.sky_r = cx.sky_g = cx.sky_b = sky; cx.W = W; cx.H = H; cx.depth = false;
    const int lane = threadIdx.x & 63;
    const uint32_t ids = ids_in[threadIdx.x >> 2];
    const int Q = (int)(ids >> 8);
    const int qy = Q / 40, qx = Q - qy * 40;
    batch_trivial<8>(cx, ids, qx * 2 + (lane & 1), qy * 2 + ((lane >> 1) & 1), true);
}
#endif
```

miniworld_amd/engine.py:

```python
from __future__ import annotations

import ctypes as C
import os
import subprocess

import numpy as np

_CSRC = os.path.join(os.path.dirname(os.path.abspath(__file__)), "csrc")
LIB_PATH = os.environ.get("MW_ENGINE_LIB") or os.path.join(_CSRC, "libmwengine.so")

ABI_VERSION = 4
MAX_REPEAT = 256
MAX_STACK = 16
STACK_PAD_RESET, STACK_PAD_ZERO = 0, 1
ENT_NONE, ENT_BOX, ENT_MESH, ENT_FRAME = 0, 1, 2, 3
POLY_ENTITY = 0x100
POLY_XF = 0x200
POLY_QUAD = 0x400
TASK_NONE, TASK_GOTO, TASK_PICKUP, TASK_PUTNEXT, TASK_SIDEWALK, TASK_SIGN, TASK_COLLECT = 0, 1, 2, 3, 4, 5, 6
GEN_NONE, GEN_HALLWAY, GEN_ONEROOM, GEN_PICKUP, GEN_MAZE, GEN_PROGRAM = 0, 1, 2, 3, 4, 5
OP_COIN, OP_DRAW_DIR, OP_PLACE, OP_FIXED, OP_BOX_SIZE, OP_COLOR, OP_APPEND = 1, 2, 3, 4, 5, 6, 7
PROG_MAX_ROOMS, PROG_MAX_TEX, PROG_MAX_OPS, PROG_MAX_ENTS = 16, 8, 48, 64
AUTORESET_OFF, AUTORESET_SAME_STEP, AUTORESET_NEXT_STEP = 0, 1, 2
OBS_HWC_U8, OBS_CWH_U8, OBS_GREY_F64 = 0, 1, 2
RNG_PHILOX, RNG_PCG64 = 0, 1
PATH_TILE, PATH_QUAD, PATH_QUAD_MESH, PATH_GENERIC = 0, 1, 2, 3

EXPORTS = [
    "mw_create", "mw_destroy", "mw_last_error", "mw_upload_texture", "mw_upload_mesh",
    "mw_set_geometry", "mw_get_geometry", "mw_set_state", "mw_get_state", "mw_set_step_params", "mw_reset",
    "mw_step", "mw_step_repeat", "mw_render", "mw_render_top", "mw_render_view", "mw_visible_ents", "mw_set_obs_layout", "mw_pcg64_draws", "mw_check", "mw_kernel_time_ms", "mw_raster_path", "mw_get_info", "mw_get_final_info", "mw_get_reset_pending", "mw_set_frame_reuse", "mw_get_frame_clean", "mw_set_frame_cache", "mw_get_frame_source", "mw_set_final_obs", "mw_get_list_lengths", "mw_debug_set_mesh_frame_seq", "mw_debug_get_slow_heads",
    "mw_set_gen_program", "mw_selftest_rcp", "mw_selftest_div", "mw_selftest_sort", "mw_selftest_q",
    "mw_selftest_sincosf",
    "mw_set_frame_stack", "mw_stack_refresh", "mw_stack_window",
    "mw_snapshot_bytes", "mw_snapshot_save", "mw_snapshot_load",
]


class MwRange(C.Structure):
    _fields_ = [("default", C.c_double), ("lo", C.c_double), ("hi", C.c_double)]

    @classmethod
    def of(cls, default, lo=None, hi=None):
        return cls(float(default), float(default if lo is None else lo), float(default if hi is None else hi))


class MwConfig(C.Structure):
    _fields_ = [
        ("abi_version", C.c_int32), ("device_id", C.c_int32), ("num_envs", C.c_int32),
        ("obs_width", C.c_int32), ("obs_height", C.c_int32), ("msaa", C.c_int32),
        ("max_ents", C.c_int32), ("max_polys", C.c_int32), ("max_segs", C.c_int32),
        ("max_visible", C.c_int32), ("shared_geometry", C.c_int32), ("task", C.c_int32),
        ("goal_ent", C.c_int32), ("goal_ent2", C.c_int32), ("num_objs", C.c_int32), ("max_episode_steps", C.c_int32),
        ("domain_rand", C.c_int32), ("generator", C.c_int32), ("autoreset", C.c_int32),
        ("agent_radius", C.c_double), ("agent_height", C.c_double), ("max_forward_step", C.c_double),
        ("forward_step", MwRange), ("forward_drift", MwRange), ("turn_step", MwRange),
        ("sky_color", MwRange * 3), ("light_pos", MwRange * 3), ("light_color", MwRange * 3),
        ("light_ambient", MwRange * 3), ("obj_color_bias", MwRange * 3),
        ("cam_height", MwRange), ("cam_fwd_disp", MwRange), ("cam_pitch", MwRange), ("cam_fov_y", MwRange),
        ("gen_args", C.c_double * 8),
        ("gen_tab", C.c_double * 12),
        ("gen_colors", C.c_double * 18),
        ("tex_nvar", C.c_int32 * 3), ("tex_var_id", (C.c_int32 * 9) * 3),
        ("tex_var_scale", ((C.c_double * 2) * 9) * 3),
        ("room_wall_height", C.c_double), ("room_no_ceiling", C.c_int32), ("rng_mode", C.c_int32),
    ]


class MwPoly(C.Structure):
    _fields_ = [("v", C.c_float * 12), ("uv", C.c_float * 8), ("n", C.c_float * 3),
                ("nv", C.c_int32), ("tex", C.c_int32), ("rgb", C.c_float * 3), ("xf", C.c_float * 4)]


POLY_DTYPE = np.dtype([("v", np.float32, (4, 3)), ("uv", np.float32, (4, 2)), ("n", np.float32, (3,)),
                       ("nv", np.int32), ("tex", np.int32), ("rgb", np.float32, (3,)), ("xf", np.float32, (4,))])
assert POLY_DTYPE.itemsize == C.sizeof(MwPoly) == 128


class MwProgRoom(C.Structure):
    _fields_ = [("nverts", C.c_int32), ("wall_tex", C.c_int32), ("floor_tex", C.c_int32), ("ceil_tex", C.c_int32),
                ("ox", C.c_double * 4), ("oz", C.c_double * 4), ("nx", C.c_double * 4), ("nz", C.c_double * 4),
                ("min_x", C.c_double), ("max_x", C.c_double), ("min_z", C.c_double), ("max_z", C.c_double), ("cdf", C.c_double)]


class MwProgOp(C.Structure):
    _fields_ = [("op", C.c_int32), ("slot", C.c_int32), ("room", C.c_int32), ("cond", C.c_int32), ("dir_mode", C.c_int32),
                ("flags", C.c_int32), ("lx", C.c_double), ("hx", C.c_double), ("lz", C.c_double), ("hz", C.c_double),
                ("dir", C.c_double), ("a", C.c_double), ("b", C.c_double)]


class MwGenProgram(C.Structure):
    _fields_ = [("n_rooms", C.c_int32), ("n_tex", C.c_int32), ("n_ops", C.c_int32), ("n_ents", C.c_int32),
                ("rooms", MwProgRoom * PROG_MAX_ROOMS),
                ("tex_nvar", C.c_int32 * PROG_MAX_TEX), ("tex_var_id", (C.c_int32 * 9) * PROG_MAX_TEX),
                ("tex_var_scale", ((C.c_double * 2) * 9) * PROG_MAX_TEX),
                ("ops", MwProgOp * PROG_MAX_OPS),
                ("ent_kind", C.c_int32 * PROG_MAX_ENTS), ("ent_mesh", C.c_int32 * PROG_MAX_ENTS), ("ent_static", C.c_int32 * PROG_MAX_ENTS),
                ("ent_pos", (C.c_double * 3) * PROG_MAX_ENTS), ("ent_dir", C.c_double * PROG_MAX_ENTS),
                ("ent_geom", (C.c_double * 9) * PROG_MAX_ENTS),
                ("colors", (C.c_double * 3) * 6), ("extent", C.c_double * 4), ("street", C.c_double * 4),
                ("sign_n", C.c_int32), ("pad", C.c_int32), ("sign_slot", C.c_int32 * 8), ("sign_reward", C.c_double * 8)]


class MwStateView(C.Structure):
    _fields_ = [(k, C.c_void_p) for k in (
        "agent_pos", "agent_dir", "cam", "light", "carrying", "step_count", "num_picked_up",
        "ent_kind", "ent_mesh", "ent_static", "ent_pos", "ent_dir", "ent_geom", "extent")]


STATE_FIELDS = {
    "agent_pos": (np.float64, lambda E: (3,)),
    "agent_dir": (np.float64, lambda E: ()),
    "cam": (np.float64, lambda E: (4,)),
    "light": (np.float64, lambda E: (12,)),
# ... 2 lines not shown
    "num_picked_up": (np.int32, lambda E: ()),
    "ent_kind": (np.int32, lambda E: (E,)),
    "ent_mesh": (np.int32, lambda E: (E,)),
    "ent_static": (np.int32, lambda E: (E,)),
    "ent_pos": (np.float64, lambda E: (E, 3)),
    "ent_dir": (np.float64, lambda E: (E,)),
    "ent_geom": (np.float64, lambda E: (E, 9)),
    "extent": (np.float64, lambda E: (4,)),
}


class EngineError(RuntimeError):
    pass


def build_library(force: bool = False) -> str:
    srcs = [os.path.join(_CSRC, f) for f in os.listdir(_CSRC) if f.endswith((".hip", ".h"))]
    srcs.append(os.path.join(_CSRC, "..", "..", "include", "mwengine.h"))
    stale = (not os.path.exists(LIB_PATH)) or any(os.path.getmtime(s) > os.path.getmtime(LIB_PATH) for s in srcs)
    if force or stale:
        r = subprocess.run([os.path.join(_CSRC, "build.sh")], capture_output=True, text=True)
        if r.returncode != 0:
            raise EngineError("building libmwengine.so failed:\n" + r.stdout + r.stderr)
    return LIB_PATH


_lib = None


def load_library():
    global _lib
    if _lib is not None:
        return _lib
    import torch
    if not os.path.exists(LIB_PATH):
        raise EngineError(
            f"{LIB_PATH} not found: the HIP engine is not built (run `python -c 'import __graft_entry__ as g; "
            "g.build()'` or miniworld_amd/csrc/build.sh).  There is no CPU fallback.")
    L = C.CDLL(LIB_PATH)
    vp, i32 = C.c_void_p, C.c_int32
    L.mw_create.argtypes = [C.POINTER(MwConfig), C.POINTER(vp)]
    L.mw_destroy.argtypes = [vp]
    L.mw_destroy.restype = None
    L.mw_last_error.argtypes = [vp]
    L.mw_last_error.restype = C.c_char_p
    L.mw_upload_texture.argtypes = [vp, i32, vp, i32, i32]
    L.mw_upload_mesh.argtypes = [vp, i32, vp, vp, vp, vp, i32, i32]
    L.mw_set_geometry.argtypes = [vp, i32, vp, i32, vp, i32]
    L.mw_get_geometry.argtypes = [vp, i32, vp, C.POINTER(i32), vp, C.POINTER(i32)]
    L.mw_set_state.argtypes = [vp, i32, i32, C.POINTER(MwStateView)]
    L.mw_get_state.argtypes = [vp, i32, i32, C.POINTER(MwStateView)]
    L.mw_set_step_params.argtypes = [vp, vp]
    L.mw_set_gen_program.argtypes = [vp, C.POINTER(MwGenProgram), vp, vp, vp, vp, i32, vp, i32]
    L.mw_reset.argtypes = [vp, vp, vp, vp]
    L.mw_step.argtypes = [vp, vp, vp, vp, vp, vp, vp, vp]
    L.mw_step_repeat.argtypes = [vp, vp, i32, vp, vp, vp, vp, vp, vp, vp]
    L.mw_render.argtypes = [vp, vp, vp, vp]
    L.mw_render_top.argtypes = [vp, vp, vp, i32, vp]
    L.mw_render_view.argtypes = [vp, i32, i32, i32, i32, i32, vp, vp, vp]
    L.mw_visible_ents.argtypes = [vp, i32, i32, vp, vp]
    L.mw_set_obs_layout.argtypes = [vp, i32]
    L.mw_set_final_obs.argtypes = [vp, vp, vp]
    L.mw_set_frame_stack.argtypes = [vp, i32, i32, vp, vp]
    L.mw_stack_refresh.argtypes = [vp, vp, vp]
    L.mw_stack_window.argtypes = [vp, C.POINTER(i32), C.POINTER(C.c_int64)]
    L.mw_snapshot_bytes.argtypes = [vp, i32]
    L.mw_snapshot_bytes.restype = C.c_int64
    L.mw_snapshot_save.argtypes = [vp, vp, i32, vp, i32, vp]
    L.mw_snapshot_load.argtypes = [vp, vp, vp, i32, vp, i32, i32, vp]
    L.mw_pcg64_draws.argtypes = [C.c_uint64, i32, vp, vp]
    L.mw_check.argtypes = [vp, vp]
    L.mw_kernel_time_ms.argtypes = [vp, i32, C.POINTER(C.c_double), C.POINTER(C.c_double), C.POINTER(C.c_int64)]
    L.mw_raster_path.argtypes = [vp]
    L.mw_get_info.argtypes = [vp, vp, vp, i32, vp]
    L.mw_get_final_info.argtypes = [vp, vp, vp, vp]
    L.mw_get_reset_pending.argtypes = [vp, vp, vp]
    L.mw_set_frame_reuse.argtypes = [vp, i32]
    L.mw_get_frame_clean.argtypes = [vp, vp, vp]
    L.mw_set_frame_cache.argtypes = [vp, i32]
    L.mw_get_frame_source.argtypes = [vp, vp, vp]
    L.mw_get_list_lengths.argtypes = [vp, i32, i32, vp, vp]
    L.mw_debug_set_mesh_frame_seq.argtypes = [vp, C.c_uint32]
    L.mw_debug_get_slow_heads.argtypes = [vp, vp, vp]
    _lib = L
    return L


def frame_reuse_allowed() -> bool:
    return os.environ.get("MW_FRAME_REUSE", "1").strip() != "0"


MAX_FRAME_CACHE = 8


def frame_cache_allowed() -> bool:
    return os.environ.get("MW_FRAME_CACHE", "1").strip() != "0"


def stack_slots(depth: int, push: int):
    p = push % depth
    return ((p + depth - 1,) if p == 0 else (p + depth - 1, p - 1)), p


def _stream_ptr(device=None):
    import torch
    return C.c_void_p(torch.cuda.current_stream(device).cuda_stream)


class Engine:

    def __init__(self, cfg: MwConfig):
        import torch
        if not torch.cuda.is_available():
            raise EngineError("no ROCm device visible: the mwengine HIP path cannot run (no CPU fallback exists)")
        self.lib = load_library()
        cfg.abi_version = ABI_VERSION
        self.cfg = cfg
        self.N = cfg.num_envs
        self.E = max(cfg.max_ents, 1)
        self.W, self.H = cfg.obs_width, cfg.obs_height
        self.obs_layout = OBS_HWC_U8
        self.device = torch.device("cuda", cfg.device_id)
        h = C.c_void_p()
        rc = self.lib.mw_create(C.byref(cfg), C.byref(h))
        if rc != 0:
            raise EngineError(f"mw_create failed ({rc}): {self.lib.mw_last_error(None).decode()}")
        self.h = h
        self.frame_reuse = False
        self.frame_cache = 0

    def _check(self, rc, what):
        if rc != 0:
            raise EngineError(f"{what} failed ({rc}): {self.lib.mw_last_error(self.h).decode()}")

    def close(self):
        if getattr(self, "h", None):
            self.lib.mw_destroy(self.h)
            self.h = None

    def __del__(self):
        try:
            self.close()
        except Exception:
            pass

    def upload_texture(self, tex_id: int, rgb_bottom_up: np.ndarray):
        a = np.ascontiguousarray(rgb_bottom_up, np.uint8)
        assert a.ndim == 3 and a.shape[2] == 3
        self._check(self.lib.mw_upload_texture(self.h, tex_id, a.ctypes.data, a.shape[1], a.shape[0]), "mw_upload_texture")

    def upload_mesh(self, mesh_id: int, verts, norms, texcs, colors, tex_id: int = -1):
        arrs = [np.ascontiguousarray(a, np.float32) for a in (verts, norms, texcs, colors)]
        n = arrs[0].shape[0]
        assert arrs[0].shape == (n, 3, 3) and arrs[1].shape == (n, 3, 3) and arrs[3].shape == (n, 3, 3)
        self._check(self.lib.mw_upload_mesh(self.h, mesh_id, arrs[0].ctypes.data, arrs[1].ctypes.data,
                                            arrs[2].ctypes.data, arrs[3].ctypes.data, n, tex_id), "mw_upload_mesh")

    def set_geometry(self, env: int, polys: np.ndarray, segs: np.ndarray):
        p = np.ascontiguousarray(polys, POLY_DTYPE)
        s = np.ascontiguousarray(segs, np.float64).reshape(-1, 4)
        self._check(self.lib.mw_set_geometry(self.h, env, p.ctypes.data, len(p), s.ctypes.data, len(s)), "mw_set_geometry")

    def get_geometry(self, env: int):
        polys = np.zeros(self.cfg.max_polys, POLY_DTYPE)
        segs = np.zeros((self.cfg.max_segs, 2, 2), np.float64)
        npoly, nseg = C.c_int32(), C.c_int32()
# ... 168 lines not shown
        ptr = lambda t: None if t is None else C.c_void_p(t.data_ptr())
        self._check(self.lib.mw_render_top(self.h, ptr(obs), ptr(depth), int(render_agent), _stream_ptr(self.device)), "mw_render_top")

    def render_view(self, env: int, width: int, height: int, msaa: int = 16, top: bool = False,
                    render_agent: bool = False, want_depth: bool = False):
        import torch
        out = torch.zeros((height, width, 3), dtype=torch.uint8, device=self.device)
        dep = torch.zeros((height, width, 1), dtype=torch.float32, device=self.device) if want_depth else None
        flags = (1 if top else 0) | (2 if render_agent else 0)
        self._check(self.lib.mw_render_view(self.h, env, flags, width, height, msaa, C.c_void_p(out.data_ptr()),
                                            None if dep is None else C.c_void_p(dep.data_ptr()), _stream_ptr(self.device)),
                    "mw_render_view")
        return (out, dep) if want_depth else out

    def set_obs_layout(self, layout: int):
        self._check(self.lib.mw_set_obs_layout(self.h, int(layout)), "mw_set_obs_layout")
        self.obs_layout = int(layout)

    def obs_buffer(self, count: int | None = None):
        import torch
        n = self.N if count is None else count
        layout = self.obs_layout
        if layout == OBS_CWH_U8:
            return torch.zeros((n, 3, self.W, self.H), dtype=torch.uint8, device=self.device)
        if layout == OBS_GREY_F64:
            return torch.zeros((n, self.H, self.W, 1), dtype=torch.float64, device=self.device)
        return torch.zeros((n, self.H, self.W, 3), dtype=torch.uint8, device=self.device)

    def visible_ents(self, first_env: int = 0, count: int | None = None):
        import torch
        count = self.N - first_env if count is None else count
        vis = torch.zeros((count, self.E), dtype=torch.uint8, device=self.device)
        self._check(self.lib.mw_visible_ents(self.h, first_env, count, C.c_void_p(vis.data_ptr()), _stream_ptr(self.device)),
                    "mw_visible_ents")
        return vis

    def check(self):
        self._check(self.lib.mw_check(self.h, _stream_ptr(self.device)), "mw_check")

    def get_info(self, health=None, ent_pos=None, ent_slot=0):
        import torch
        for t, dt, shape in ((health, torch.int32, (self.N,)), (ent_pos, torch.float64, (self.N, 3))):
            if t is not None:
                assert t.is_cuda and t.dtype == dt and tuple(t.shape) == shape and t.is_contiguous()
        self._check(self.lib.mw_get_info(self.h, health.data_ptr() if health is not None else None,
                                         ent_pos.data_ptr() if ent_pos is not None else None, int(ent_slot), _stream_ptr(self.device)), "mw_get_info")

    def get_final_info(self, health=None, goal_pos=None):
        import torch
        for t, dt, shape in ((health, torch.int32, (self.N,)), (goal_pos, torch.float64, (self.N, 3))):
            if t is not None:
                assert t.is_cuda and t.dtype == dt and tuple(t.shape) == shape and t.is_contiguous()
        self._check(self.lib.mw_get_final_info(self.h, health.data_ptr() if health is not None else None,
                                               goal_pos.data_ptr() if goal_pos is not None else None, _stream_ptr(self.device)), "mw_get_final_info")

    def get_reset_pending(self, out=None):
        import torch
        if out is None:
            out = torch.zeros(self.N, dtype=torch.uint8, device=self.device)
        assert out.is_cuda and out.dtype == torch.uint8 and tuple(out.shape) == (self.N,) and out.is_contiguous()
        self._check(self.lib.mw_get_reset_pending(self.h, out.data_ptr(), _stream_ptr(self.device)), "mw_get_reset_pending")
        return out

    def set_frame_reuse(self, on: bool):
        on = bool(on) and frame_reuse_allowed()
        self._check(self.lib.mw_set_frame_reuse(self.h, int(on)), "mw_set_frame_reuse")
        self.frame_reuse = on
        return on

    def set_frame_cache(self, slots: int):
        slots = int(slots) if frame_cache_allowed() else 0
        self._check(self.lib.mw_set_frame_cache(self.h, slots), "mw_set_frame_cache")
        self.frame_cache = slots
        return slots

    def get_frame_source(self, out=None):
        import torch
        if out is None:
            out = torch.zeros(self.N, dtype=torch.uint8, device=self.device)
        assert out.is_cuda and out.dtype == torch.uint8 and tuple(out.shape) == (self.N,) and out.is_contiguous()
        self._check(self.lib.mw_get_frame_source(self.h, out.data_ptr(), _stream_ptr(self.device)), "mw_get_frame_source")
        return out

    def get_frame_clean(self, out=None):
        import torch
        if out is None:
            out = torch.zeros(self.N, dtype=torch.uint8, device=self.device)
        assert out.is_cuda and out.dtype == torch.uint8 and tuple(out.shape) == (self.N,) and out.is_contiguous()
        self._check(self.lib.mw_get_frame_clean(self.h, out.data_ptr(), _stream_ptr(self.device)), "mw_get_frame_clean")
        return out

    def list_lengths(self):
        out = np.zeros(self.N, np.int32)
        self._check(self.lib.mw_get_list_lengths(self.h, 0, self.N, out.ctypes.data, _stream_ptr(self.device)), "mw_get_list_lengths")
        return out

    def raster_path(self):
        return int(self.lib.mw_raster_path(self.h))

    def kernel_time_ms(self, reset=0):
        r, s, n = C.c_double(), C.c_double(), C.c_int64()
        self._check(self.lib.mw_kernel_time_ms(self.h, reset, C.byref(r), C.byref(s), C.byref(n)), "mw_kernel_time_ms")
        return r.value, s.value, n.value



def default_ranges() -> dict:
    return {
        "sky_color": ([0.25, 0.82, 1.0], [0.1, 0.1, 0.1], [1.0, 1.0, 1.0]),
        "light_pos": ([0, 2.5, 0], [-40, 2.5, -40], [40, 5, 40]),
        "light_color": ([0.7, 0.7, 0.7], [0.45, 0.45, 0.45], [0.8, 0.8, 0.8]),
        "light_ambient": ([0.45, 0.45, 0.45], [0.35, 0.35, 0.35], [0.55, 0.55, 0.55]),
        "obj_color_bias": ([0, 0, 0], [-0.2, -0.2, -0.2], [0.2, 0.2, 0.2]),
        "forward_step": (0.15, 0.12, 0.17),
        "forward_drift": (0.0, -0.05, 0.05),
        "turn_step": (15.0, 10.0, 20.0),
        "cam_pitch": (0.0, -5.0, 5.0),
        "cam_fov_y": (60.0, 55.0, 65.0),
        "cam_height": (1.5, 1.45, 1.55),
        "cam_fwd_disp": (0.0, -0.05, 0.10),
    }


def fill_ranges(cfg: MwConfig, ranges: dict | None = None):
    r = default_ranges() if ranges is None else ranges
    for name in ("forward_step", "forward_drift", "turn_step", "cam_pitch", "cam_fov_y", "cam_height", "cam_fwd_disp"):
        setattr(cfg, name, MwRange.of(*r[name]))
    for name in ("sky_color", "light_pos", "light_color", "light_ambient", "obj_color_bias"):
        d, lo, hi = r[name]
        arr = getattr(cfg, name)
        for k in range(3):
            arr[k] = MwRange.of(d[k], lo[k], hi[k])
    cfg.max_forward_step = float(r["forward_step"][2])
```

Before: 15.70 million.

## Plan frame reuse and cache hits before geometry and fold copies into geom

Adds a frame-plan kernel that decides per env whether the frame is left as is, copied from the frame cache, or drawn. It compacts the drawn envs and the cached copies into two lists. The geometry kernel then runs only over the drawn envs, with extra waves doing the cache copies, and the raster kernel walks the compacted draw list. Before, every env's geometry was computed and each raster block checked for reuse or a cache hit on its own. This avoids geometry and raster launches for envs that skip drawing, at the cost of an extra kernel, atomics, and a memset per step.

```diff
diff --git a/include/mwengine.h b/include/mwengine.h
--- a/include/mwengine.h
+++ b/include/mwengine.h
@@ -232,6 +232,7 @@
 
 int mw_set_frame_cache(mw_engine *e, int32_t slots);
 int mw_get_frame_source(mw_engine *e, uint8_t *d_out, void *stream);
+int mw_debug_get_frame_keys(mw_engine *e, uint64_t *host_keys, uint64_t *host_table, void *stream);
 
 int mw_get_list_lengths(mw_engine *e, int32_t first_env, int32_t count, int32_t *host_out, void *stream);
 
diff --git a/miniworld_amd/csrc/mw_engine.hip b/miniworld_amd/csrc/mw_engine.hip
--- a/miniworld_amd/csrc/mw_engine.hip
+++ b/miniworld_amd/csrc/mw_engine.hip
@@ -160,6 +160,7 @@
     uint8_t *final_obs = nullptr;
     float *final_depth = nullptr;
     int32_t *d_final_list = nullptr;
+    int32_t *d_plan = nullptr;
     bool frame_reuse = false;
     struct { uint8_t *obs = nullptr; float *depth = nullptr; int layout = 0; bool valid = false; } held;
     struct {
@@ -300,6 +301,13 @@
     return fixed8 ? MW_PAIR(mw_geom) : MW_PAIR(mw_geom_any);
 }
 
+auto geom_plan_kernel_of(int L, int msaa) -> decltype(&mw_geom_plan_kernel)
+{
+    const bool fixed8 = msaa == 8;
+    if (L == 64) return fixed8 ? mw_geom_big_plan_kernel : mw_geom_big_any_plan_kernel;
+    return fixed8 ? mw_geom_plan_kernel : mw_geom_any_plan_kernel;
+}
+
 auto tile_kernel_of(bool big, bool depth, bool general, bool ragged, bool mesh, bool first)
 {
     if (mesh) {
@@ -601,7 +609,7 @@
     const int32_t *list;
     uint8_t *obs; float *depth; hipStream_t st; bool reuse;
     int fc_slots;
-    uint8_t *source;
+    const int32_t *plan;
     RasterPath p;
     MeshFrame mf;
 };
@@ -624,7 +632,13 @@
     if (frame == FRAME_TERMINAL)
         hipLaunchKernelGGL(mw_final_list_kernel, dim3(1), dim3(1024), 0, f.st, N, (const uint8_t *)a.reset_pending, a.pending_remove, e->d_final_list);
     const int L = geom_lanes(e), epw = 64 / L;
-    launch(geom_kernel_of(L, e->cfg.msaa), f.list, dim3((N + epw - 1) / epw), dim3(64), 0, f.st, a, f.view_flags, e->cfg.msaa, L, N);
+    if (f.plan) {
+        const MwFcArgs *fc = f.fc_slots ? (const MwFcArgs *)e->fc.d_args.get() : nullptr;
+        hipLaunchKernelGGL(mw_frame_plan_kernel, dim3((N + 7) / 8), dim3(64), 0, f.st, a, (int)f.reuse, fc, e->d_plan);
+        hipLaunchKernelGGL(geom_plan_kernel_of(L, e->cfg.msaa), dim3(mw_plan_grid(N, epw)), dim3(64), 0, f.st, a, f.view_flags, e->cfg.msaa, L, N,
+                           MwPlanCopy{f.plan, f.obs, f.depth, fc});
+    } else
+        launch(geom_kernel_of(L, e->cfg.msaa), f.list, dim3((N + epw - 1) / epw), dim3(64), 0, f.st, a, f.view_flags, e->cfg.msaa, L, N);
     if (do_step && e->cfg.task == MW_TASK_COLLECT)
         hipLaunchKernelGGL(e->cfg.rng_mode == MW_RNG_PCG64 ? mw_collect_respawn_pcg_kernel : mw_collect_respawn_kernel, dim3((N + 63) / 64), dim3(64), 0, f.st, a);
 }
@@ -665,7 +679,7 @@
     launch(f.p.quad4 ? MW_PAIR(mw_rasterq4) : MW_PAIR(mw_rasterq), f.list, dim3(e->cfg.num_envs), dim3(MWQ_THREADS), (size_t)lds, st, a.N, a.W, a.H, a.max_vis,
            a.tiles_x, a.n_tiles, (const float *)a.rec_raster, (const float *)a.rec_shade, (const float *)a.rec_cull,
            (const int32_t *)a.nvis, (const float *)a.envhdr, a.texels, f.obs, f.depth, raster_flags(e, part, 0u, f.reuse), e->texel_bytes, e->d_k2q_prof,
-           (const uint8_t *)a.frame_clean, f.fc_slots ? (const MwFcArgs *)e->fc.d_args.get() : nullptr, f.source);
+           f.fc_slots ? (const MwFcArgs *)e->fc.d_args.get() : nullptr, f.plan ? MW_PLAN_DRAW(f.plan) : nullptr);
 }
 
 void launch_tiles(const mw_engine *e, const Frame &f, int part, hipStream_t st)
@@ -725,7 +739,6 @@
     const int N = e->cfg.num_envs;
     Frame f{e->args, view_flags, frame == FRAME_LIST ? e->d_final_list : nullptr, d_obs, d_depth, st, reuse, 0, nullptr, raster_path(e, d_depth != nullptr), {}};
     if (plain && do_step && f.p.path == MW_PATH_QUAD) {
-        f.source = f.a.fc_source;
         if (e->fc.slots > 0 && e->fc.frames && !e->have_meshes && e->dbg_flags == 0 && e->obs_layout == MW_OBS_HWC_U8 && e->cfg.task != MW_TASK_COLLECT) {
             if (d_depth && !e->fc.depth) {
                 if (const int rc = dev_alloc(e, e->fc.depth, (size_t)N * e->fc.slots * f.a.W * f.a.H, false)) return rc;
@@ -743,6 +756,11 @@
                 e->fc.dirty = false;
             }
             f.fc_slots = e->fc.slots;
+        }
+        if (reuse || f.fc_slots) {
+            if (N > (1 << MW_PLAN_ENV_BITS)) return fail(e, MW_E_CAPACITY, "%d envs: an entry of the frame plan's lists holds %d bits of env", N, MW_PLAN_ENV_BITS);
+            f.plan = e->d_plan;
+            HIP_TRY(e, hipMemsetAsync(e->d_plan, 0, 2 * sizeof(int32_t), st));
         }
     }
     f.a.step_override = e->use_step_override ? e->d_step_override : nullptr;
@@ -879,6 +897,7 @@
     ALLOC(a.nvis, N); ALLOC(a.envhdr, (size_t)MW_ENVHDR * N); ALLOC(a.status, 1);
     ALLOC(e->d_reward_scratch, N); ALLOC(e->d_flag_scratch, 2 * (size_t)N); ALLOC(e->d_action_scratch, N);
     ALLOC(e->d_final_list, 1 + (size_t)N);
+    ALLOC(e->d_plan, MW_PLAN_WORDS(N));
     ALLOC(e->stack.flags, 2 * (size_t)N);
     ALLOC(e->d_mask, N); ALLOC(e->d_step_override, 3 * (size_t)N);
 #ifdef MW_PERF_HOOKS
@@ -1646,6 +1665,18 @@
     return MW_OK;
 }
 
+int mw_debug_get_frame_keys(mw_engine *e, uint64_t *host_keys, uint64_t *host_table, void *stream)
+{
+    if (!e || !host_keys) return fail(e, MW_E_INVALID, "null argument");
+    if (host_table && !(e->fc.slots > 0 && e->fc.meta)) return fail(e, MW_E_INVALID, "mw_debug_get_frame_keys: this engine has no frame cache");
+    ON_DEVICE(e);
+    const size_t N = (size_t)e->cfg.num_envs;
+    HIP_TRY(e, hipStreamSynchronize((hipStream_t)stream));
+    HIP_TRY(e, hipMemcpy(host_keys, e->args.fc_key, N * MW_FC_KEY_WORDS * sizeof(uint64_t), hipMemcpyDeviceToHost));
+    if (host_table) HIP_TRY(e, hipMemcpy(host_table, e->fc.meta.get(), N * MW_FC_META_WORDS(e->fc.slots) * sizeof(uint64_t), hipMemcpyDeviceToHost));
+    return MW_OK;
+}
+
 int mw_get_frame_clean(mw_engine *e, uint8_t *d_out, void *stream)
 {
     if (!e) return MW_E_INVALID;
diff --git a/miniworld_amd/csrc/mw_frame_plan.h b/miniworld_amd/csrc/mw_frame_plan.h
--- /dev/null
+++ b/miniworld_amd/csrc/mw_frame_plan.h
@@ -0,0 +1,121 @@
+#pragma once
+#include <stddef.h>
+#include <stdint.h>
+#include "mw_hd.h"
+
+#ifndef MW_FC_KEY_WORDS
+#define MW_FC_KEY_WORDS 10
+#endif
+
+#define MW_PLAN_DRAWN 0
+#define MW_PLAN_LEFT 1
+#define MW_PLAN_COPIED 2
+
+#define MW_PLAN_WORDS(N) (2 + 2 * (size_t)(N))
+#define MW_PLAN_DRAW(plan) ((plan) + 1)
+#define MW_PLAN_COPY_COUNT(plan) ((plan)[0])
+#define MW_PLAN_COPY(plan, N) ((plan) + 2 + (N))
+#define MW_PLAN_ENV_BITS 24
+#define MW_PLAN_ENV(entry) ((int)((uint32_t)(entry) & ((1u << MW_PLAN_ENV_BITS) - 1u)))
+#define MW_PLAN_SLOT(entry) ((uint32_t)(entry) >> MW_PLAN_ENV_BITS)
+#define MW_PLAN_ENTRY(env, slot) ((int32_t)((uint32_t)(env) | ((uint32_t)(slot) << MW_PLAN_ENV_BITS)))
+
+MW_HD bool mw_fc_key_match(const uint64_t *key, const uint64_t *slot_key)
+{
+    bool eq = true;
+    for (int w = 0; w < MW_FC_KEY_WORDS; ++w) eq = eq && key[w] == slot_key[w];
+    return eq;
+}
+
+MW_HD int mw_frame_verdict(bool clean, uint32_t match)
+{
+    if (clean) return MW_PLAN_LEFT;
+    for (int j = 0; j < 32; ++j)
+        if ((match >> j) & 1u) return MW_PLAN_COPIED + j;
+    return MW_PLAN_DRAWN;
+}
+
+MW_HD int mw_frame_verdict_of(bool reuse, uint8_t frame_clean, const uint64_t *key, const uint64_t *meta, int slots)
+{
+    uint32_t match = 0u;
+    if (meta)
+        for (int j = 0; j < slots; ++j)
+            if (mw_fc_key_match(key, meta + 2 + MW_FC_KEY_WORDS * j)) match |= 1u << j;
+    return mw_frame_verdict(reuse && frame_clean != 0, match);
+}
+
+MW_HD uint32_t mw_frame_victim(const uint64_t *meta, int slots)
+{
+    const uint32_t v = (uint32_t)meta[0], last = (uint32_t)(slots - 1);
+    return v < last ? v : last;
+}
+
+MW_HD int mw_plan_grid(int N, int epw) { return (N + epw - 1) / epw + 1; }
+MW_HD int mw_plan_geom_waves(int n_draw, int epw) { return (n_draw + epw - 1) / epw; }
+struct MwPlanRole {
+    bool copy;
+    int first, stride;
+};
+MW_HD MwPlanRole mw_plan_role(int wave, int grid, int n_draw, int epw)
+{
+    const int n_geom = mw_plan_geom_waves(n_draw, epw);
+    return MwPlanRole{wave >= n_geom, wave - n_geom, grid - n_geom};
+}
+
+#ifdef __HIPCC__
+#include "mw_device.h"
+struct MwPlanCopy {
+    const int32_t *plan;
+    uint8_t *obs;
+    float *depth;
+    const MwFcArgs *fc;
+};
+
+template <typename T>
+__device__ inline void mw_plan_copy_units(T *__restrict__ dst, const T *__restrict__ src, int n, int lane)
+{
+    constexpr int U = 6;
+    for (int base = 0; base < n; base += 64 * U) {
+        T v[U];
+#pragma unroll
+        for (int u = 0; u < U; ++u) {
+            const int i = base + u * 64 + lane;
+            if (i < n) v[u] = src[i];
+        }
+#pragma unroll
+        for (int u = 0; u < U; ++u) {
+            const int i = base + u * 64 + lane;
+            if (i < n) dst[i] = v[u];
+        }
+    }
+}
+
+__device__ inline void mw_plan_copy_wave(const MwPlanCopy &cp, int N, int W, int H, const MwPlanRole &r, int lane)
+{
+    const int n_copy = MW_PLAN_COPY_COUNT(cp.plan);
+    if (n_copy <= 0) return;
+    const int32_t *copies = MW_PLAN_COPY(cp.plan, N);
+    const int slots = cp.fc->slots, npix = W * H, fbytes = npix * 3;
+    for (int i = r.first; i < n_copy; i += r.stride) {
+        const int32_t entry = copies[i];
+        const int env = MW_PLAN_ENV(entry);
+        const size_t slot = (size_t)env * slots + MW_PLAN_SLOT(entry);
+        const uint8_t *src = cp.fc->frames + slot * fbytes;
+        uint8_t *dst = cp.obs + (size_t)env * fbytes;
+        if ((reinterpret_cast<uintptr_t>(dst) & 15u) == 0u)
+            mw_plan_copy_units(reinterpret_cast<uint4 *>(dst), reinterpret_cast<const uint4 *>(src), fbytes / 16, lane);
+        else if ((reinterpret_cast<uintptr_t>(dst) & 3u) == 0u)
+            mw_plan_copy_units(reinterpret_cast<uint32_t *>(dst), reinterpret_cast<const uint32_t *>(src), fbytes / 4, lane);
+        else
+            mw_plan_copy_units(dst, src, fbytes, lane);
+        if (cp.depth) {
+            const float *zs = cp.fc->depth + slot * npix;
+            float *zd = cp.depth + (size_t)env * npix;
+            if ((reinterpret_cast<uintptr_t>(zd) & 15u) == 0u)
+                mw_plan_copy_units(reinterpret_cast<float4 *>(zd), reinterpret_cast<const float4 *>(zs), npix / 4, lane);
+            else
+                mw_plan_copy_units(zd, zs, npix, lane);
+        }
+    }
+}
+#endif
diff --git a/miniworld_amd/csrc/mw_frame_plan.hip b/miniworld_amd/csrc/mw_frame_plan.hip
--- /dev/null
+++ b/miniworld_amd/csrc/mw_frame_plan.hip
@@ -0,0 +1,43 @@
+#include <hip/hip_runtime.h>
+#include "mw_kernels.h"
+
+static_assert(MW_FC_MAX_SLOTS <= 8, "a lane per slot in a group of eight");
+
+__device__ inline int plan_append(int32_t *count, bool on, int lane)
+{
+    const uint64_t m = __builtin_amdgcn_ballot_w64(on);
+    int base = 0;
+    if (lane == 0 && m) base = atomicAdd(count, (int)__popcll(m));
+    base = __builtin_amdgcn_readfirstlane(base);
+    return base + (int)__popcll(m & ((1ull << lane) - 1ull));
+}
+
+extern "C" __global__ __launch_bounds__(64) void mw_frame_plan_kernel(MwArgs a, int reuse, const MwFcArgs *__restrict__ fc, int32_t *__restrict__ plan)
+{
+    const int lane = threadIdx.x, grp = lane >> 3, j = lane & 7;
+    const int env = (int)blockIdx.x * 8 + grp;
+    const bool live = env < a.N;
+    const int slots = fc ? fc->slots : 0;
+    const uint64_t *meta = fc ? fc->meta + (size_t)(live ? env : 0) * MW_FC_META_WORDS(slots) : nullptr;
+    bool eq = false;
+    if (live && j < slots) eq = mw_fc_key_match(fc->key + (size_t)env * MW_FC_KEY_WORDS, meta + 2 + MW_FC_KEY_WORDS * j);
+    const uint32_t match = (uint32_t)(__builtin_amdgcn_ballot_w64(eq) >> (grp * 8)) & 0xFFu;
+    const bool writer = live && j == 0;
+    int verdict = MW_PLAN_DRAWN;
+    if (writer) {
+        verdict = mw_frame_verdict(reuse != 0 && a.frame_clean[env] != 0, match);
+        a.fc_source[env] = (uint8_t)verdict;
+    }
+    const bool draw = writer && verdict == MW_PLAN_DRAWN, copy = writer && verdict >= MW_PLAN_COPIED;
+    const int at_draw = plan_append(plan + 1, draw, lane);
+    const int at_copy = plan_append(plan + 0, copy, lane);
+    if (draw) MW_PLAN_DRAW(plan)[1 + at_draw] = MW_PLAN_ENTRY(env, slots ? mw_frame_victim(meta, slots) : 0u);
+    if (copy) MW_PLAN_COPY(plan, a.N)[at_copy] = MW_PLAN_ENTRY(env, verdict - MW_PLAN_COPIED);
+    if (writer && verdict != MW_PLAN_DRAWN && a.task != MW_TASK_COLLECT) {
+        const int rs = a.pending_remove[env];
+        if (rs >= 0) {
+            a.ekind[(size_t)rs * a.N + env] = MW_ENT_NONE;
+            a.pending_remove[env] = MW_REMOVE_APPLIED;
+        }
+    }
+}
diff --git a/miniworld_amd/csrc/mw_geom.hip b/miniworld_amd/csrc/mw_geom.hip
--- a/miniworld_amd/csrc/mw_geom.hip
+++ b/miniworld_amd/csrc/mw_geom.hip
@@ -149,9 +149,17 @@
 
 }
 
-template <bool BIG, int SFIX, bool SUB = false>
-__device__ inline void geom_body(const MwArgs &a, int view_flags, int S_, int L, int n_env, const int32_t *__restrict__ list = nullptr)
-{
+template <bool BIG, int SFIX, bool SUB = false, bool PLAN = false>
+__device__ inline void geom_body(const MwArgs &a, int view_flags, int S_, int L, int n_env, const int32_t *__restrict__ list = nullptr,
+                                 const MwPlanCopy *cp = nullptr)
+{
+    if constexpr (PLAN) {
+        const MwPlanRole role = mw_plan_role((int)blockIdx.x, (int)gridDim.x, list[0], 64 / L);
+        if (role.copy) {
+            mw_plan_copy_wave(*cp, a.N, a.W, a.H, role, (int)threadIdx.x);
+            return;
+        }
+    }
     const int S = SFIX ? SFIX : S_;
     struct ClipSlot { mwgl::ClipVert l[2][MWGL_MAX_CLIP_VERTS]; float pad[4]; };
     __shared__ ClipSlot s_clip[kClipSlots];
@@ -182,7 +190,8 @@
     }
     const int rel = (int)blockIdx.x * epw + grp;
     const bool live = rel < n_env;
-    const int env = SUB ? list[1 + (live ? rel : n_env - 1)] : a.env_base + (live ? rel : n_env - 1);
+    const int listed = SUB ? list[1 + (live ? rel : n_env - 1)] : 0;
+    const int env = SUB ? (PLAN ? MW_PLAN_ENV(listed) : listed) : a.env_base + (live ? rel : n_env - 1);
     const int set = a.shared_geom ? 0 : env;
     const bool top = (view_flags & 1) != 0, proxy = (view_flags & 4) != 0, ms = S > 1;
     constexpr int kWallPf = BIG ? 4 : 1;
@@ -1120,7 +1129,8 @@
 #endif
 #define MW_GEOM_PAIR(stem, bounds, ...)                                                                                        \
     extern "C" __global__ bounds void stem##_kernel(MW_GEOM_ARGS) { geom_body<__VA_ARGS__, false>(a, view_flags, S, L, n_env); } \
-    extern "C" __global__ bounds void stem##_sub_kernel(MW_GEOM_ARGS, const int32_t *list) { geom_body<__VA_ARGS__, true>(a, view_flags, S, L, n_env, list); }
+    extern "C" __global__ bounds void stem##_sub_kernel(MW_GEOM_ARGS, const int32_t *list) { geom_body<__VA_ARGS__, true>(a, view_flags, S, L, n_env, list); } \
+    extern "C" __global__ bounds void stem##_plan_kernel(MW_GEOM_ARGS, MwPlanCopy cp) { geom_body<__VA_ARGS__, true, true>(a, view_flags, S, L, n_env, MW_PLAN_DRAW(cp.plan), &cp); }
 MW_GEOM_PAIR(mw_geom, __launch_bounds__(64) MW_GEOM_OCC, false, 8)
 MW_GEOM_PAIR(mw_geom_big, __launch_bounds__(64) MW_GEOM_OCC, true, 8)
 MW_GEOM_PAIR(mw_geom_any, __launch_bounds__(64), false, 0)
diff --git a/miniworld_amd/csrc/mw_kernels.h b/miniworld_amd/csrc/mw_kernels.h
--- a/miniworld_amd/csrc/mw_kernels.h
+++ b/miniworld_amd/csrc/mw_kernels.h
@@ -1,5 +1,6 @@
 #pragma once
 #include "mw_device.h"
+#include "mw_frame_plan.h"
 #include "mw_snapshot.h"
 
 #define MW_KERNEL_PAIR(stem, ...)                          \
@@ -28,11 +29,16 @@
 extern "C" __global__ void mw_final_install_pcg_kernel(MwArgs a, const int32_t *__restrict__ list);
 extern "C" __global__ void mw_take_spare_kernel(MwArgs a, const uint8_t *__restrict__ mask, int force_all);
 
+extern "C" __global__ void mw_frame_plan_kernel(MwArgs a, int reuse, const MwFcArgs *__restrict__ fc, int32_t *__restrict__ plan);
+
 #define MW_GEOM_ARGS MwArgs a, int view_flags, int S, int L, int n_env
-MW_KERNEL_PAIR(mw_geom, MW_GEOM_ARGS);
-MW_KERNEL_PAIR(mw_geom_big, MW_GEOM_ARGS);
-MW_KERNEL_PAIR(mw_geom_any, MW_GEOM_ARGS);
-MW_KERNEL_PAIR(mw_geom_big_any, MW_GEOM_ARGS);
+#define MW_GEOM_KERNELS(stem)            \
+    MW_KERNEL_PAIR(stem, MW_GEOM_ARGS);  \
+    extern "C" __global__ void stem##_plan_kernel(MW_GEOM_ARGS, MwPlanCopy cp)
+MW_GEOM_KERNELS(mw_geom);
+MW_GEOM_KERNELS(mw_geom_big);
+MW_GEOM_KERNELS(mw_geom_any);
+MW_GEOM_KERNELS(mw_geom_big_any);
 
 #define MW_RASTER_REUSE 0x10000
 
@@ -67,7 +73,7 @@
     const float *__restrict__ rec_raster, const float *__restrict__ rec_shade, const float *__restrict__ rec_cull, \
     const int32_t *__restrict__ nvis_arr, const float *__restrict__ envhdr, const uint32_t *__restrict__ texels, \
     uint8_t *__restrict__ obs, float *__restrict__ depth, int dbg, int texel_bytes, unsigned long long *__restrict__ prof, \
-    const uint8_t *__restrict__ frame_clean, const MwFcArgs *__restrict__ fc, uint8_t *__restrict__ frame_source
+    const MwFcArgs *__restrict__ fc, const int32_t *__restrict__ draw
 MW_KERNEL_PAIR(mw_rasterq, MWQ_ARGS);
 MW_KERNEL_PAIR(mw_rasterq4, MWQ_ARGS);
 extern "C" int mw_rasterq_lds_bytes(int S, int W, int H, int n_tiles, int depth);
diff --git a/miniworld_amd/csrc/mw_rasterq.hip b/miniworld_amd/csrc/mw_rasterq.hip
--- a/miniworld_amd/csrc/mw_rasterq.hip
+++ b/miniworld_amd/csrc/mw_rasterq.hip
@@ -481,61 +481,23 @@
     const float *__restrict__ rec_raster, const float *__restrict__ rec_shade, const float *__restrict__ rec_cull,
     const int32_t *__restrict__ nvis_arr, const float *__restrict__ envhdr, const uint32_t *__restrict__ texels,
     uint8_t *__restrict__ obs, float *__restrict__ depth, int dbg, int texel_bytes, unsigned long long *__restrict__ prof,
-    const uint8_t *__restrict__ frame_clean, const MwFcArgs *__restrict__ fc, uint8_t *__restrict__ frame_source,
-    const int32_t *__restrict__ list = nullptr)
+    const MwFcArgs *__restrict__ fc, const int32_t *__restrict__ draw, const int32_t *__restrict__ list = nullptr)
 {
     extern __shared__ __attribute__((aligned(16))) unsigned char smem[];
     typedef QRec<S> R;
     int env = blockIdx.x;
+    uint32_t fc_victim = 0u;
     if (SUB) {
         if (env >= list[0]) return;
         env = list[1 + env];
+    } else if (draw) {
+        if (env >= draw[0]) return;
+        const int32_t entry = draw[1 + env];
+        env = MW_PLAN_ENV(entry);
+        fc_victim = MW_PLAN_SLOT(entry);
     } else if (env >= N) return;
-    if (!SUB && (dbg & MW_RASTER_REUSE) && frame_clean[env]) {
-        if (frame_source && threadIdx.x == 0) frame_source[env] = 1;
-        return;
-    }
     const int tid = threadIdx.x, lane = tid & 63, wave = tid >> 6;
     const bool has_depth = depth != nullptr;
-    uint32_t fc_victim = 0u;
-    if (!SUB && fc) {
-        const int fc_slots = fc->slots;
-        const uint64_t *meta = fc->meta + (size_t)env * MW_FC_META_WORDS(fc_slots);
-        const uint4 *cur = reinterpret_cast<const uint4 *>(fc->key + (size_t)env * MW_FC_KEY_WORDS);
-        bool eq = false;
-        uint4 k = make_uint4(0u, 0u, 0u, 0u);
-        if (lane < fc_slots * (MW_FC_KEY_WORDS / 2)) {
-            const uint4 c = cur[lane % (MW_FC_KEY_WORDS / 2)];
-            k = reinterpret_cast<const uint4 *>(meta + 2)[lane];
-            eq = k.x == c.x && k.y == c.y && k.z == c.z && k.w == c.w;
-        } else if (lane == 63) k = reinterpret_cast<const uint4 *>(meta)[0];
-        const uint64_t m = __builtin_amdgcn_ballot_w64(eq);
-        int hit = -1;
-        for (int j = fc_slots - 1; j >= 0; --j)
-            if (((m >> (j * (MW_FC_KEY_WORDS / 2))) & 31ull) == 31ull) hit = j;
-        if (hit >= 0) {
-            const int fbytes = W * H * 3;
-            const uint8_t *src = fc->frames + ((size_t)env * fc_slots + hit) * fbytes;
-            uint8_t *dst = obs + (size_t)env * fbytes;
-            if ((reinterpret_cast<uintptr_t>(dst) & 15u) == 0u)
-                for (int i = tid; i < fbytes / 16; i += MWQ_THREADS) reinterpret_cast<uint4 *>(dst)[i] = reinterpret_cast<const uint4 *>(src)[i];
-            else if ((reinterpret_cast<uintptr_t>(dst) & 3u) == 0u)
-                for (int i = tid; i < fbytes / 4; i += MWQ_THREADS) reinterpret_cast<uint32_t *>(dst)[i] = reinterpret_cast<const uint32_t *>(src)[i];
-            else
-                for (int i = tid; i < fbytes; i += MWQ_THREADS) dst[i] = src[i];
-            if (has_depth) {
-                const float *zs = fc->depth + ((size_t)env * fc_slots + hit) * (W * H);
-                float *zd = depth + (size_t)env * (W * H);
-                if ((reinterpret_cast<uintptr_t>(zd) & 15u) == 0u)
-                    for (int i = tid; i < W * H / 4; i += MWQ_THREADS) reinterpret_cast<float4 *>(zd)[i] = reinterpret_cast<const float4 *>(zs)[i];
-                else
-                    for (int i = tid; i < W * H; i += MWQ_THREADS) zd[i] = zs[i];
-            }
-            if (frame_source && tid == 0) frame_source[env] = (uint8_t)(2 + hit);
-            return;
-        }
-        fc_victim = min((uint32_t)__builtin_amdgcn_readlane((int)k.x, 63), (uint32_t)(fc_slots - 1));
-    }
     const QPlan pl = q_plan(S, W, H, n_tiles, has_depth);
     float4 *s_rec = reinterpret_cast<float4 *>(smem + pl.rec);
     uint8_t *s_frame = smem + pl.frame;
@@ -938,7 +900,7 @@
 
 }
 
-#define MWQ_FWD N, W, H, max_vis, tiles_x, n_tiles, rec_raster, rec_shade, rec_cull, nvis_arr, envhdr, texels, obs, depth, dbg, texel_bytes, prof, frame_clean, fc, frame_source
+#define MWQ_FWD N, W, H, max_vis, tiles_x, n_tiles, rec_raster, rec_shade, rec_cull, nvis_arr, envhdr, texels, obs, depth, dbg, texel_bytes, prof, fc, draw
 #define MWQ_PAIR(stem, bounds, ...)                                                                          \
     extern "C" __global__ bounds void stem##_kernel(MWQ_ARGS) { rasterq_body<__VA_ARGS__, false>(MWQ_FWD); } \
     extern "C" __global__ bounds void stem##_sub_kernel(MWQ_ARGS, const int32_t *__restrict__ list) { rasterq_body<__VA_ARGS__, true>(MWQ_FWD, list); }
diff --git a/miniworld_amd/engine.py b/miniworld_amd/engine.py
--- a/miniworld_amd/engine.py
+++ b/miniworld_amd/engine.py
@@ -29,7 +29,7 @@
 EXPORTS = [
     "mw_create", "mw_destroy", "mw_last_error", "mw_upload_texture", "mw_upload_mesh",
     "mw_set_geometry", "mw_get_geometry", "mw_set_state", "mw_get_state", "mw_set_step_params", "mw_reset",
-    "mw_step", "mw_step_repeat", "mw_render", "mw_render_top", "mw_render_view", "mw_visible_ents", "mw_set_obs_layout", "mw_pcg64_draws", "mw_check", "mw_kernel_time_ms", "mw_raster_path", "mw_get_info", "mw_get_final_info", "mw_get_reset_pending", "mw_set_frame_reuse", "mw_get_frame_clean", "mw_set_frame_cache", "mw_get_frame_source", "mw_set_final_obs", "mw_get_list_lengths", "mw_debug_set_mesh_frame_seq", "mw_debug_get_slow_heads",
+    "mw_step", "mw_step_repeat", "mw_render", "mw_render_top", "mw_render_view", "mw_visible_ents", "mw_set_obs_layout", "mw_pcg64_draws", "mw_check", "mw_kernel_time_ms", "mw_raster_path", "mw_get_info", "mw_get_final_info", "mw_get_reset_pending", "mw_set_frame_reuse", "mw_get_frame_clean", "mw_set_frame_cache", "mw_get_frame_source", "mw_set_final_obs", "mw_get_list_lengths", "mw_debug_set_mesh_frame_seq", "mw_debug_get_slow_heads", "mw_debug_get_frame_keys",
     "mw_set_gen_program", "mw_selftest_rcp", "mw_selftest_div", "mw_selftest_sort", "mw_selftest_q",
     "mw_selftest_sincosf",
     "mw_set_frame_stack", "mw_stack_refresh", "mw_stack_window",
@@ -198,6 +198,7 @@
     L.mw_get_list_lengths.argtypes = [vp, i32, i32, vp, vp]
     L.mw_debug_set_mesh_frame_seq.argtypes = [vp, C.c_uint32]
     L.mw_debug_get_slow_heads.argtypes = [vp, vp, vp]
+    L.mw_debug_get_frame_keys.argtypes = [vp, vp, vp, vp]
     _lib = L
     return L
 
@@ -532,6 +533,13 @@
         self._check(self.lib.mw_get_frame_source(self.h, out.data_ptr(), _stream_ptr(self.device)), "mw_get_frame_source")
         return out
 
+    def debug_frame_keys(self):
+        keys = np.zeros((self.N, 10), np.uint64)
+        table = np.zeros((self.N, 2 + 10 * self.frame_cache), np.uint64) if self.frame_cache else None
+        self._check(self.lib.mw_debug_get_frame_keys(self.h, keys.ctypes.data, table.ctypes.data if table is not None else None,
+                                                     _stream_ptr(self.device)), "mw_debug_get_frame_keys")
+        return keys, table
+
     def get_frame_clean(self, out=None):
         import torch
         if out is None:
```

Result: no change. 15.85 million (median of 2 runs) (+1.0%).
